# wing02/MyLdpcCppApi

Measured on AMD Instinct MI355X. Metric: decoded Mbit/s (info bits), DVB-S2 N=64800 rate-1/2, 50 iters, higher is better.
Workload: dtype f32; 1 GPU; DVB-S2-profile (64800,32400) rate-1/2 (seeded IRA table with the standard's structure, E=226799), batch 4096 frames per GPU, 50 iterations, sum-product fp32 (probability domain), all-zero codeword + AWGN sigma=0.95 (no frame converges), early termination on, inputs resident in HBM; global_batch=4096, frames_per_gpu=4096, algo=sp, frames_per_launch=4096, parallelism=frames sharded over 1 GPU(s), all-gather of decoded bytes, frames_converged=0

## Files before the change

### include/ldpc_hip.h

```cpp
#ifndef LDPC_HIP_H_
#define LDPC_HIP_H_

#include <stddef.h>
#include <stdint.h>

#ifdef __cplusplus
extern "C" {
#endif

#define LDPC_HIP_ABI_VERSION 3

enum ldpc_status {
    LDPC_OK = 0,
    LDPC_ERR_ARG = 1,
    LDPC_ERR_HIP = 2,
    LDPC_ERR_NOMEM = 3,
    LDPC_ERR_UNSUPPORTED = 4,
    LDPC_ERR_STATE = 5
};

enum ldpc_algo {
    LDPC_ALGO_SP = 0,
    LDPC_ALGO_MS = 1,
    LDPC_ALGO_LAYERED = 2,
    LDPC_ALGO_MS_FUSED = 3,
    LDPC_ALGO_LAYERED_HOST = 4
};

enum ldpc_msg_dtype { LDPC_MSG_F32 = 0, LDPC_MSG_F16 = 1 };

enum ldpc_host_input { LDPC_HOST_INPUT_AUTO = 0, LDPC_HOST_INPUT_STAGED = 1, LDPC_HOST_INPUT_LOCK_PAGES = 2 };

enum ldpc_pack_mode {
    LDPC_PACK_BYTES = 0,
    LDPC_PACK_BITS = 1
};

typedef struct ldpc_graph ldpc_graph;
typedef struct ldpc_decoder ldpc_decoder;

typedef struct ldpc_decoder_config {
    uint32_t struct_size;
    int32_t K;
    int32_t max_batch;
    int32_t algo;
    int32_t msg_dtype;
    int32_t max_iter;
    float llr_scale;
    int32_t early_term;
    int32_t device;
    int32_t layer_rows;
    int32_t pack_mode;
    int32_t frames_per_lane;
    int32_t poll_interval;
    int32_t tune_flags;
    int32_t tune_rows_per_wave;
    int32_t tune_cols_per_wave;
    int32_t tune_link_rows;
    int32_t tune_compact;
    int32_t tune_ldsp_grid;
    int32_t tune_ldsp_shape;
    int32_t tune_place;
    int32_t host_input;
    int32_t host_copy_threads;
    int32_t tune_q_order;
    float ms_scale;
    float ms_offset;
} ldpc_decoder_config;

enum ldpc_tune_field {
    LDPC_TUNE_FUSED = 0,
    LDPC_TUNE_LDSP = 2,
    LDPC_TUNE_LDSP_EXT = 4,
    LDPC_TUNE_LDSP_PACK = 6,
    LDPC_TUNE_LINK_NARROW = 8,
    LDPC_TUNE_CHECK_WIDE = 10,
    LDPC_TUNE_SYN_XCD = 12,
    LDPC_TUNE_FUSED_PACK = 14,
    LDPC_TUNE_FUSED_LOOP = 16,
    LDPC_TUNE_DEVICE_TAIL = 18,
    LDPC_TUNE_MERGE = 20,
    LDPC_TUNE_LINK_DEEP = 22,
    LDPC_TUNE_LINK_HALF = 24,
    LDPC_TUNE_LINK_GUIDED = 26,
    LDPC_TUNE_TILES_FIRST = 28
};
#define LDPC_TUNE_ON(field) (1 << (field))
#define LDPC_TUNE_OFF(field) (2 << (field))

typedef struct ldpc_decode_stats {
    int32_t iterations_launched;
    int32_t batch_time;
    int64_t frames;
    int64_t frames_converged;
    float ms_total;
    float ms_check;
    float ms_var;
    float ms_other;
    int32_t launches_check;
    int32_t launches_var;
    int64_t frame_rounds;
} ldpc_decode_stats;

int ldpc_abi_version(void);
const char *ldpc_last_error(void);
int ldpc_device_count(int *count);

int ldpc_graph_create(const int32_t *rows, const int32_t *cols, int64_t E, int32_t M, int32_t N,
                      ldpc_graph **out);
int ldpc_graph_destroy(ldpc_graph *g);
int ldpc_graph_info(const ldpc_graph *g, int32_t *M, int32_t *N, int64_t *E, int32_t *max_row_deg,
                    int32_t *max_col_deg);

void ldpc_decoder_config_init(ldpc_decoder_config *cfg);
int ldpc_decoder_create(const ldpc_graph *g, const ldpc_decoder_config *cfg, ldpc_decoder **out);
int ldpc_decoder_create_multi(const ldpc_graph *g, const ldpc_decoder_config *cfg, const int32_t *devices,
                              int32_t n_devices, ldpc_decoder **out);
int ldpc_decoder_destroy(ldpc_decoder *d);
int ldpc_shard_range(int64_t frames, int32_t part, int32_t parts, int32_t unit, int64_t *lo, int64_t *hi);

int ldpc_decode(ldpc_decoder *d, const float *llr_host, int64_t frames, uint8_t *out_host,
                int64_t out_bytes, int32_t *iters);

int ldpc_decode_device(ldpc_decoder *d, const float *llr_dev, int64_t frames, uint8_t *out_dev,
                       int64_t out_bytes, int32_t *iters_dev, void *stream);

int64_t ldpc_out_bytes(int32_t K, int64_t frames, int32_t pack_mode);

int ldpc_decoder_set_timing(ldpc_decoder *d, int enable);
int ldpc_decoder_stats(ldpc_decoder *d, ldpc_decode_stats *stats);

typedef struct ldpc_kernel_time {
    int32_t phase;
    int32_t degree;
    int32_t launches;
    float ms_total;
    int64_t bytes_total;
    char name[64];
    int64_t bytes_moved;
} ldpc_kernel_time;
int ldpc_decoder_kernel_times(ldpc_decoder *d, ldpc_kernel_time *out, int32_t capacity,
                              int32_t *count);

int ldpc_decoder_link_form(ldpc_decoder *d, int32_t *form, int32_t *calibrated, float ms[3]);

int ldpc_decoder_placement(ldpc_decoder *d, int32_t *candidates, int32_t *kept, float ms[16]);
int ldpc_decoder_array_addresses(ldpc_decoder *d, uint64_t out[4]);

int ldpc_decoder_set_tap(ldpc_decoder *d, int32_t iter);
int ldpc_decoder_dump(ldpc_decoder *d, int32_t which, float *host_out, int64_t count);

int ldpc_awgn_device(float *llr_dev, int64_t frames, int32_t N, const uint8_t *bits_dev, float sd,
                     uint64_t seed, int64_t first_frame, int32_t device, void *stream);
int ldpc_count_errors_device(const uint8_t *out_dev, const uint8_t *ref_dev, int64_t frames,
                             int64_t bytes_per_frame, int64_t errors[3], int32_t device, void *stream);

typedef struct ldpc_encoder ldpc_encoder;
enum ldpc_code_format {
    LDPC_CODE_PACKED = 0,
    LDPC_CODE_BITS = 1
};
enum ldpc_parity_kind { LDPC_PARITY_DUAL_DIAGONAL = 1, LDPC_PARITY_STAIRCASE = 2 };
int ldpc_parity_structure(const ldpc_graph *g, int32_t K, int32_t block_rows, int32_t out[8]);
int ldpc_encoder_create(const ldpc_graph *g, int32_t K, int32_t block_rows, int32_t max_frames, int32_t device,
                        ldpc_encoder **out);
int ldpc_encoder_destroy(ldpc_encoder *e);
int ldpc_encode_device(ldpc_encoder *e, const uint8_t *src_dev, int64_t src_bytes, int64_t frames, uint8_t *code_dev,
                       int64_t code_bytes, int32_t format, void *stream);
int ldpc_encode(ldpc_encoder *e, const uint8_t *src_host, int64_t src_bytes, uint8_t *code_host, int64_t code_bytes);
int64_t ldpc_code_bytes(int32_t N, int64_t frames, int32_t format);

int ldpc_hbm_probe_device(int32_t device, int64_t bytes, int32_t reps, double *copy_gbs, double *by_policy);
int ldpc_hbm_sustained_device(int32_t device, int64_t bytes, int32_t milliseconds, double *copy_gbs);

int ldpc_host_block_plan(uint64_t base, int64_t frames, int32_t N, int32_t max_batch, int64_t group, uint64_t out[6]);
int ldpc_host_locked_ranges(int64_t *live, int64_t *stale);

#ifdef __cplusplus
}
#endif
#endif
```

### myldpccppapi_amd/_lib.py

```python
import ctypes
import os
import sys

_HERE = os.path.dirname(os.path.abspath(__file__))
LIB_PATH = os.environ.get("LDPC_HIP_LIB") or os.path.join(_HERE, "libldpc_hip.so")
_lib = None


class LdpcError(RuntimeError):
    def __init__(self, code, message):
        super().__init__("ldpc_hip error %d: %s" % (code, message))
        self.code = code


class DecoderConfig(ctypes.Structure):
    _fields_ = [("struct_size", ctypes.c_uint32), ("K", ctypes.c_int32),
                ("max_batch", ctypes.c_int32), ("algo", ctypes.c_int32),
                ("msg_dtype", ctypes.c_int32), ("max_iter", ctypes.c_int32),
                ("llr_scale", ctypes.c_float), ("early_term", ctypes.c_int32),
                ("device", ctypes.c_int32), ("layer_rows", ctypes.c_int32),
                ("pack_mode", ctypes.c_int32), ("frames_per_lane", ctypes.c_int32),
                ("poll_interval", ctypes.c_int32),
                ("tune_flags", ctypes.c_int32), ("tune_rows_per_wave", ctypes.c_int32),
                ("tune_cols_per_wave", ctypes.c_int32), ("tune_link_rows", ctypes.c_int32),
                ("tune_compact", ctypes.c_int32), ("tune_ldsp_grid", ctypes.c_int32),
                ("tune_ldsp_shape", ctypes.c_int32), ("tune_place", ctypes.c_int32),
                ("host_input", ctypes.c_int32),
                ("host_copy_threads", ctypes.c_int32), ("tune_q_order", ctypes.c_int32),
                ("ms_scale", ctypes.c_float), ("ms_offset", ctypes.c_float)]


class DecodeStats(ctypes.Structure):
    _fields_ = [("iterations_launched", ctypes.c_int32), ("batch_time", ctypes.c_int32),
                ("frames", ctypes.c_int64), ("frames_converged", ctypes.c_int64),
                ("ms_total", ctypes.c_float), ("ms_check", ctypes.c_float),
                ("ms_var", ctypes.c_float), ("ms_other", ctypes.c_float),
                ("launches_check", ctypes.c_int32), ("launches_var", ctypes.c_int32),
                ("frame_rounds", ctypes.c_int64)]


class KernelTime(ctypes.Structure):
    _fields_ = [("phase", ctypes.c_int32), ("degree", ctypes.c_int32), ("launches", ctypes.c_int32),
                ("ms_total", ctypes.c_float), ("bytes_total", ctypes.c_int64), ("name", ctypes.c_char * 64),
                ("bytes_moved", ctypes.c_int64)]


EXPORTS = (
    "ldpc_abi_version", "ldpc_last_error", "ldpc_device_count", "ldpc_graph_create",
    "ldpc_graph_destroy", "ldpc_graph_info", "ldpc_decoder_config_init", "ldpc_decoder_create",
    "ldpc_decoder_create_multi", "ldpc_shard_range", "ldpc_decoder_destroy", "ldpc_decode", "ldpc_decode_device", "ldpc_out_bytes",
    "ldpc_decoder_set_timing", "ldpc_decoder_stats", "ldpc_decoder_kernel_times", "ldpc_decoder_set_tap",
    "ldpc_decoder_dump", "ldpc_awgn_device", "ldpc_count_errors_device", "ldpc_hbm_probe_device", "ldpc_hbm_sustained_device",
    "ldpc_host_block_plan", "ldpc_host_locked_ranges", "ldpc_decoder_link_form", "ldpc_decoder_placement", "ldpc_decoder_array_addresses",
    "ldpc_parity_structure", "ldpc_encoder_create", "ldpc_encoder_destroy", "ldpc_encode_device", "ldpc_encode", "ldpc_code_bytes",
)


def load():
    global _lib
    if _lib is not None:
        return _lib
    if not os.path.exists(LIB_PATH):
        raise OSError("%s not built: run `python -c 'import __graft_entry__ as g; g.build()'` "
                      "or `make -C myldpccppapi_amd/csrc`" % LIB_PATH)
    if "torch" not in sys.modules:
        try:
            import torch
        except Exception:
            pass
    L = ctypes.CDLL(LIB_PATH, mode=ctypes.RTLD_GLOBAL)
    i32p = ctypes.POINTER(ctypes.c_int32)
    i64p = ctypes.POINTER(ctypes.c_int64)
    vp = ctypes.c_void_p
    L.ldpc_abi_version.restype = ctypes.c_int
    L.ldpc_last_error.restype = ctypes.c_char_p
    L.ldpc_device_count.argtypes = [ctypes.POINTER(ctypes.c_int)]
    L.ldpc_graph_create.argtypes = [i32p, i32p, ctypes.c_int64, ctypes.c_int32, ctypes.c_int32,
                                    ctypes.POINTER(vp)]
    L.ldpc_graph_destroy.argtypes = [vp]
    L.ldpc_graph_info.argtypes = [vp, i32p, i32p, i64p, i32p, i32p]
    L.ldpc_decoder_config_init.argtypes = [ctypes.POINTER(DecoderConfig)]
    L.ldpc_decoder_config_init.restype = None
    L.ldpc_decoder_create.argtypes = [vp, ctypes.POINTER(DecoderConfig), ctypes.POINTER(vp)]
    L.ldpc_decoder_create_multi.argtypes = [vp, ctypes.POINTER(DecoderConfig), i32p, ctypes.c_int32,
                                            ctypes.POINTER(vp)]
    L.ldpc_shard_range.argtypes = [ctypes.c_int64, ctypes.c_int32, ctypes.c_int32, ctypes.c_int32, i64p, i64p]
    L.ldpc_decoder_destroy.argtypes = [vp]
    L.ldpc_decode.argtypes = [vp, vp, ctypes.c_int64, vp, ctypes.c_int64, vp]
    L.ldpc_decode_device.argtypes = [vp, vp, ctypes.c_int64, vp, ctypes.c_int64, vp, vp]
    L.ldpc_out_bytes.argtypes = [ctypes.c_int32, ctypes.c_int64, ctypes.c_int32]
    L.ldpc_out_bytes.restype = ctypes.c_int64
    L.ldpc_decoder_set_timing.argtypes = [vp, ctypes.c_int]
    L.ldpc_decoder_stats.argtypes = [vp, ctypes.POINTER(DecodeStats)]
    L.ldpc_decoder_kernel_times.argtypes = [vp, ctypes.POINTER(KernelTime), ctypes.c_int32, i32p]
    L.ldpc_decoder_set_tap.argtypes = [vp, ctypes.c_int32]
    L.ldpc_decoder_dump.argtypes = [vp, ctypes.c_int32, vp, ctypes.c_int64]
    L.ldpc_awgn_device.argtypes = [vp, ctypes.c_int64, ctypes.c_int32, vp, ctypes.c_float, ctypes.c_uint64,
                                   ctypes.c_int64, ctypes.c_int32, vp]
    L.ldpc_count_errors_device.argtypes = [vp, vp, ctypes.c_int64, ctypes.c_int64, i64p, ctypes.c_int32, vp]
    L.ldpc_hbm_sustained_device.argtypes = [ctypes.c_int32, ctypes.c_int64, ctypes.c_int32, ctypes.POINTER(ctypes.c_double)]
    L.ldpc_hbm_probe_device.argtypes = [ctypes.c_int32, ctypes.c_int64, ctypes.c_int32,
                                        ctypes.POINTER(ctypes.c_double), ctypes.POINTER(ctypes.c_double)]
    L.ldpc_host_block_plan.argtypes = [ctypes.c_uint64, ctypes.c_int64, ctypes.c_int32, ctypes.c_int32, ctypes.c_int64,
                                       ctypes.POINTER(ctypes.c_uint64)]
    L.ldpc_host_locked_ranges.argtypes = [i64p, i64p]
    L.ldpc_decoder_array_addresses.argtypes = [vp, ctypes.POINTER(ctypes.c_uint64)]
    L.ldpc_decoder_placement.argtypes = [vp, i32p, i32p, ctypes.POINTER(ctypes.c_float)]
    L.ldpc_decoder_link_form.argtypes = [vp, i32p, i32p, ctypes.POINTER(ctypes.c_float)]
    L.ldpc_parity_structure.argtypes = [vp, ctypes.c_int32, ctypes.c_int32, i32p]
    L.ldpc_encoder_create.argtypes = [vp, ctypes.c_int32, ctypes.c_int32, ctypes.c_int32, ctypes.c_int32, ctypes.POINTER(vp)]
    L.ldpc_encoder_destroy.argtypes = [vp]
    L.ldpc_encode_device.argtypes = [vp, vp, ctypes.c_int64, ctypes.c_int64, vp, ctypes.c_int64, ctypes.c_int32, vp]
    L.ldpc_encode.argtypes = [vp, vp, ctypes.c_int64, vp, ctypes.c_int64]
    L.ldpc_code_bytes.argtypes = [ctypes.c_int32, ctypes.c_int64, ctypes.c_int32]
    L.ldpc_code_bytes.restype = ctypes.c_int64
    _lib = L
    return L


def check(rc):
    if rc != 0:
        raise LdpcError(rc, load().ldpc_last_error().decode("utf-8", "replace"))
```

### myldpccppapi_amd/capi.py

```python
import ctypes

import numpy as np

from . import _lib
from ._lib import DecoderConfig, DecodeStats, LdpcError

ALGO_SP, ALGO_MS, ALGO_LAYERED, ALGO_MS_FUSED, ALGO_LAYERED_HOST = 0, 1, 2, 3, 4
MSG_F32, MSG_F16 = 0, 1
PACK_BYTES, PACK_BITS = 0, 1
CODE_PACKED, CODE_BITS = 0, 1
CODE_FORMATS = {"packed": CODE_PACKED, "bits": CODE_BITS}
PARITY_KINDS = {1: "dual_diagonal", 2: "staircase"}
HOST_INPUT = {"auto": 0, "staged": 1, "lock_pages": 2}
ALGOS = {"sp": ALGO_SP, "ms": ALGO_MS, "layered": ALGO_LAYERED, "ms_fused": ALGO_MS_FUSED,
         "layered_host": ALGO_LAYERED_HOST}

TUNE_FIELDS = {"fused": 0, "ldsp": 2, "ldsp_ext": 4, "ldsp_pack": 6, "link_narrow": 8, "check_wide": 10,
               "syn_xcd": 12, "fused_pack": 14, "fused_loop": 16, "device_tail": 18, "merge": 20, "link_deep": 22, "link_half": 24,
               "link_guided": 26, "tiles_first": 28}
TUNE_INTS = ("rows_per_wave", "cols_per_wave", "link_rows", "compact", "ldsp_grid", "ldsp_per_cu", "ldsp_waves", "place", "q_order")


def apply_tune(cfg, tune):
    flags, shape = 0, 0
    for k, v in (tune or {}).items():
        if k in TUNE_FIELDS:
            if v is not None:
                flags |= (1 if v else 2) << TUNE_FIELDS[k]
        elif k == "ldsp_per_cu":
            shape |= int(v) & 255
        elif k == "ldsp_waves":
            shape |= (int(v) & 255) << 8
        elif k in TUNE_INTS:
            setattr(cfg, "tune_" + k, int(v))
        else:
            raise KeyError("unknown tuning field %r" % k)
    cfg.tune_flags, cfg.tune_ldsp_shape = flags, shape


def hbm_probe(device=0, nbytes=1 << 30, reps=5, by_policy=False):
    g = ctypes.c_double(0.0)
    two = (ctypes.c_double * 2)(0.0, 0.0)
    _lib.check(_lib.load().ldpc_hbm_probe_device(int(device), int(nbytes), int(reps), ctypes.byref(g), two))
    return (g.value, two[0], two[1]) if by_policy else g.value


def hbm_sustained(device=0, nbytes=1 << 30, milliseconds=300):
    g = ctypes.c_double(0.0)
    _lib.check(_lib.load().ldpc_hbm_sustained_device(int(device), int(nbytes), int(milliseconds), ctypes.byref(g)))
    return g.value


def tune_from_env(env=None):
    import os
    env = os.environ if env is None else env
    t = {}
    for name, key in (("FUSED", "fused"), ("LDSP", "ldsp"), ("LDSP_EXT", "ldsp_ext"), ("LDSP_PACK", "ldsp_pack"),
                      ("LINK_NARROW", "link_narrow"), ("CHECK_WIDE", "check_wide"), ("SYN_XCD", "syn_xcd"),
                      ("FUSED_LOOP", "fused_loop"), ("DEVICE_TAIL", "device_tail"), ("MERGE", "merge"), ("LINK_DEEP", "link_deep"), ("LINK_HALF", "link_half"),
                      ("LINK_GUIDED", "link_guided"), ("TILES_FIRST", "tiles_first")):
        if "LDPC_TUNE_" + name in env:
            t[key] = int(env["LDPC_TUNE_" + name]) != 0
    if "LDPC_TUNE_NO_PACK" in env:
        t["fused_pack"] = False
    for name, key in (("RPW", "rows_per_wave"), ("CPW", "cols_per_wave"), ("LDSP_GRID", "ldsp_grid"),
                      ("LDSP_PER_CU", "ldsp_per_cu"), ("LDSP_WAVES", "ldsp_waves")):
        if "LDPC_TUNE_" + name in env:
            t[key] = int(env["LDPC_TUNE_" + name])
    for name, key in (("LINK_RPW", "link_rows"), ("COMPACT", "compact")):
        if "LDPC_TUNE_" + name in env:
            v = int(env["LDPC_TUNE_" + name])
            t[key] = v if v > 0 else -1
    return t


def shard_range(frames, part, parts, unit=1):
    lo, hi = ctypes.c_int64(), ctypes.c_int64()
    _lib.check(_lib.load().ldpc_shard_range(int(frames), int(part), int(parts), int(unit),
                                            ctypes.byref(lo), ctypes.byref(hi)))
    return lo.value, hi.value


def host_block_plan(base, frames, N, max_batch, group):
    out = (ctypes.c_uint64 * 6)()
    _lib.check(_lib.load().ldpc_host_block_plan(int(base), int(frames), int(N), int(max_batch), int(group), out))
    return tuple(int(x) for x in out)


def host_locked_ranges():
    a, b = ctypes.c_int64(-1), ctypes.c_int64(-1)
    _lib.check(_lib.load().ldpc_host_locked_ranges(ctypes.byref(a), ctypes.byref(b)))
    return a.value, b.value


def device_count():
    n = ctypes.c_int(0)
    rc = _lib.load().ldpc_device_count(ctypes.byref(n))
    return n.value if rc == 0 else 0


def out_bytes(K, frames, pack_mode=PACK_BYTES):
    return int(_lib.load().ldpc_out_bytes(K, frames, pack_mode))


def code_bytes(N, frames, fmt="packed"):
    return int(_lib.load().ldpc_code_bytes(int(N), int(frames), CODE_FORMATS.get(fmt, fmt)))


def parity_structure(graph, K, block_rows=0):
    out = (ctypes.c_int32 * 8)()
    _lib.check(_lib.load().ldpc_parity_structure(graph._h, int(K), int(block_rows), out))
    return dict(kind=PARITY_KINDS[out[0]], c=out[1], x=out[2], a=out[3], b=out[4], ext_rows=out[5], z=out[6])


class Graph:

    def __init__(self, rows, cols, M, N):
        L = _lib.load()
        self.rows = np.ascontiguousarray(rows, np.int32)
        self.cols = np.ascontiguousarray(cols, np.int32)
        if self.rows.shape != self.cols.shape or self.rows.ndim != 1:
            raise ValueError("rows and cols must be 1-D arrays of equal length")
        self.M, self.N, self.E = int(M), int(N), int(self.rows.size)
        self._h = ctypes.c_void_p()
        i32p = ctypes.POINTER(ctypes.c_int32)
        _lib.check(L.ldpc_graph_create(self.rows.ctypes.data_as(i32p), self.cols.ctypes.data_as(i32p),
                                       self.E, self.M, self.N, ctypes.byref(self._h)))

    def info(self):
        L = _lib.load()
        M, N, rd, cd = (ctypes.c_int32() for _ in range(4))
        E = ctypes.c_int64()
        _lib.check(L.ldpc_graph_info(self._h, ctypes.byref(M), ctypes.byref(N), ctypes.byref(E),
                                     ctypes.byref(rd), ctypes.byref(cd)))
        return dict(M=M.value, N=N.value, E=E.value, max_row_deg=rd.value, max_col_deg=cd.value)

    def close(self):
        h, self._h = getattr(self, "_h", None), None
        if h and _lib is not None and _lib._lib is not None:
            _lib._lib.ldpc_graph_destroy(h)

    def __del__(self):
        try:
            self.close()
        except Exception:
            pass


class Decoder:

    def __init__(self, graph, K, max_batch, algo="sp", max_iter=40, llr_scale=8.0, early_term=True,
                 device=0, layer_rows=0, pack_mode=PACK_BYTES, frames_per_lane=0, poll_interval=0,
                 msg_dtype=MSG_F32, tune=None, devices=None, host_input="auto", host_copy_threads=0,
                 ms_scale=0.0, ms_offset=0.0):
        L = _lib.load()
        cfg = DecoderConfig()
        L.ldpc_decoder_config_init(ctypes.byref(cfg))
        cfg.K, cfg.max_batch = int(K), int(max_batch)
        cfg.algo = ALGOS[algo] if isinstance(algo, str) else int(algo)
        cfg.msg_dtype = {"f32": MSG_F32, "f16": MSG_F16}.get(msg_dtype, msg_dtype)
        cfg.max_iter, cfg.llr_scale = int(max_iter), float(llr_scale)
        cfg.early_term, cfg.device, cfg.layer_rows = int(bool(early_term)), int(device), int(layer_rows)
        cfg.pack_mode, cfg.frames_per_lane, cfg.poll_interval = int(pack_mode), int(frames_per_lane), int(poll_interval)
        apply_tune(cfg, tune)
        cfg.host_input = HOST_INPUT[host_input] if isinstance(host_input, str) else int(host_input)
        cfg.host_copy_threads = int(host_copy_threads)
        cfg.ms_scale, cfg.ms_offset = float(ms_scale), float(ms_offset)
        self.cfg = cfg
        self.graph = graph
        self.K, self.N, self.E = int(K), graph.N, graph.E
        self._h = ctypes.c_void_p()
        if devices is None:
            _lib.check(L.ldpc_decoder_create(graph._h, ctypes.byref(cfg), ctypes.byref(self._h)))
        else:
            devs = (ctypes.c_int32 * len(devices))(*[int(x) for x in devices])
            _lib.check(L.ldpc_decoder_create_multi(graph._h, ctypes.byref(cfg), devs, len(devices),
                                                   ctypes.byref(self._h)))

    def decode(self, llr, want_iters=True):
        L = _lib.load()
        llr = np.ascontiguousarray(llr, np.float32).reshape(-1, self.N)
        frames = llr.shape[0]
        out = np.zeros(out_bytes(self.K, frames, self.cfg.pack_mode), np.uint8)
        iters = np.zeros(frames, np.int32)
        _lib.check(L.ldpc_decode(self._h, llr.ctypes.data, frames, out.ctypes.data, out.size,
                                 iters.ctypes.data if want_iters else None))
        return out, iters

    def decode_device(self, llr_ptr, frames, out_ptr, out_nbytes, iters_ptr=None, stream=None):
        _lib.check(_lib.load().ldpc_decode_device(self._h, llr_ptr, frames, out_ptr, out_nbytes,
                                                  iters_ptr, stream))

    def set_timing(self, enable=True):
        _lib.check(_lib.load().ldpc_decoder_set_timing(self._h, int(enable)))

    def stats(self):
        st = DecodeStats()
        _lib.check(_lib.load().ldpc_decoder_stats(self._h, ctypes.byref(st)))
        return {f: getattr(st, f) for f, _ in st._fields_}

    def kernel_times(self):
        arr = (_lib.KernelTime * 64)()
        n = ctypes.c_int32(0)
        _lib.check(_lib.load().ldpc_decoder_kernel_times(self._h, arr, 64, ctypes.byref(n)))
        return [dict(name=arr[i].name.decode(), phase=arr[i].phase, degree=arr[i].degree,
                     launches=arr[i].launches, ms_total=arr[i].ms_total, bytes_total=arr[i].bytes_total,
                     bytes_moved=arr[i].bytes_moved)
                for i in range(n.value)]

    def link_form(self):
        form, cal = ctypes.c_int32(-1), ctypes.c_int32(0)
        ms = (ctypes.c_float * 3)()
        _lib.check(_lib.load().ldpc_decoder_link_form(self._h, ctypes.byref(form), ctypes.byref(cal), ms))
        if form.value < 0:
            return None
        return {"form": ("wide", "narrow", "half")[form.value], "chosen_by_measurement": bool(cal.value),
                "ms_per_launch": {"wide": round(ms[0], 4), "narrow": round(ms[1], 4), "half": round(ms[2], 4)}}

    def placement(self):
        n, kept = ctypes.c_int32(0), ctypes.c_int32(0)
        ms = (ctypes.c_float * 16)()
        _lib.check(_lib.load().ldpc_decoder_placement(self._h, ctypes.byref(n), ctypes.byref(kept), ms))
        if n.value == 0:
            return None
        return {"candidates_ms": [round(ms[i], 4) for i in range(n.value)], "kept": kept.value}

    def array_addresses(self):
        a = (ctypes.c_uint64 * 4)()
        _lib.check(_lib.load().ldpc_decoder_array_addresses(self._h, a))
        return {"Q": int(a[0]), "R": int(a[1]), "chan": int(a[2]), "hard": int(a[3])}

    def set_tap(self, it):
        _lib.check(_lib.load().ldpc_decoder_set_tap(self._h, int(it)))

    def dump(self, which, frames):
        per = self.N if which in (2, 3) else self.E
        a = np.empty((frames, per), np.float32)
        _lib.check(_lib.load().ldpc_decoder_dump(self._h, which, a.ctypes.data, a.size))
        return a

    def close(self):
        h, self._h = getattr(self, "_h", None), None
        if h and _lib is not None and _lib._lib is not None:
            _lib.check(_lib._lib.ldpc_decoder_destroy(h))

    def __del__(self):
        try:
            self.close()
        except Exception:
            pass


class Encoder:

    def __init__(self, graph, K, block_rows=0, max_frames=4096, device=0):
        L = _lib.load()
        self.graph, self.K, self.N = graph, int(K), graph.N
        self.block_rows, self.max_frames, self.device = int(block_rows), int(max_frames), int(device)
        self._h = ctypes.c_void_p()
        _lib.check(L.ldpc_encoder_create(graph._h, self.K, self.block_rows, self.max_frames, self.device,
                                         ctypes.byref(self._h)))

    def structure(self):
        return parity_structure(self.graph, self.K, self.block_rows)

    def encode(self, src_bytes):
        src = np.ascontiguousarray(np.frombuffer(bytes(src_bytes), np.uint8) if isinstance(src_bytes, (bytes, bytearray))
                                   else src_bytes, np.uint8).reshape(-1)
        frames = 1
        while frames * self.K // 8 < src.size:
            frames += 1
        out = np.zeros(code_bytes(self.N, frames, "packed"), np.uint8)
        _lib.check(_lib.load().ldpc_encode(self._h, src.ctypes.data, src.size, out.ctypes.data, out.size))
        return out

    def encode_device(self, src_ptr, src_nbytes, frames, code_ptr, code_nbytes, fmt="bits", stream=None):
        _lib.check(_lib.load().ldpc_encode_device(self._h, src_ptr, int(src_nbytes), int(frames), code_ptr,
                                                  int(code_nbytes), CODE_FORMATS.get(fmt, fmt), stream))

    def close(self):
        h, self._h = getattr(self, "_h", None), None
        if h and _lib is not None and _lib._lib is not None:
            _lib.check(_lib._lib.ldpc_encoder_destroy(h))

    def __del__(self):
        try:
            self.close()
        except Exception:
            pass
```

### myldpccppapi_amd/csrc/flood_kernels.hpp

```cpp
#pragma once

#include <hip/hip_runtime.h>
#include <stdint.h>

#include "ldpc_expf.h"

namespace ldpc {

constexpr int kAlgoSP = 0;
constexpr int kAlgoMS = 1;
constexpr int kAlgoMSC = 2;
constexpr int kCompactCapacity = 512;
constexpr int kLastCapacity = 64;
constexpr int kBlock = 256;
constexpr int kWavesPerBlock = 4;
constexpr int kMaxUnrolledDegree = 16;
constexpr int kMaxUnrolledCheckDegreeMS = 32;

#ifndef LDPC_NT_LOAD
#define LDPC_NT_LOAD 1
#endif
#ifndef LDPC_NT_STORE
#define LDPC_NT_STORE 1
#endif
// ... 58 lines not shown
    const vh4 t = ld_stream(reinterpret_cast<const vh4 *>(p));
    d[0] = (float)t.x; d[1] = (float)t.y; d[2] = (float)t.z; d[3] = (float)t.w;
}
template <int V> __device__ __forceinline__ void vstore(hf *p, const float (&s)[V]);
template <> __device__ __forceinline__ void vstore<1>(hf *p, const float (&s)[1]) { st_stream(p, (hf)s[0]); }
template <> __device__ __forceinline__ void vstore<2>(hf *p, const float (&s)[2])
{
    vh2 t; t.x = (hf)s[0]; t.y = (hf)s[1];
    st_stream(reinterpret_cast<vh2 *>(p), t);
}
template <> __device__ __forceinline__ void vstore<4>(hf *p, const float (&s)[4])
{
    vh4 t; t.x = (hf)s[0]; t.y = (hf)s[1]; t.z = (hf)s[2]; t.w = (hf)s[3];
    st_stream(reinterpret_cast<vh4 *>(p), t);
}

__device__ __forceinline__ int wave_id_in_block()
{
    return __builtin_amdgcn_readfirstlane((int)(threadIdx.x >> 6));
}

template <int V> __device__ __forceinline__ bool tile_finished(const uint64_t *done, int tile)
{
    bool all = true;
#pragma unroll
    for (int v = 0; v < V; ++v) all = all && (done[(size_t)tile * V + v] == ~0ull);
    return all;
}

struct TailRef {
    const int32_t *state;
    int32_t base_tile;
    int32_t n_tiles;
};

template <int V> __device__ __forceinline__ int tile_select(const TailRef &t, const uint64_t *done, int row)
{
    int tile = row;
    if (t.state && __builtin_amdgcn_readfirstlane(t.state[0])) {
        if (row >= t.n_tiles) return -1;
        tile = t.base_tile + row;
    }
    return tile_finished<V>(done, tile) ? -1 : tile;
}


struct CheckArgs {
    const void *__restrict__ Q;
    void *__restrict__ R;
    const int32_t *__restrict__ cls_e0;
    const uint64_t *__restrict__ done;
    int64_t E;
    int32_t n_rows;
    int32_t rows_per_wave;
    int32_t degree;
    float ms_scale = 1.0f;
    TailRef tail;
    int32_t tiles_first = 0;
    float ms_offset = 0.0f;
    const void *__restrict__ first_chan = nullptr;
    const int32_t *__restrict__ edge_col = nullptr;
    int32_t N = 0;
    const int32_t *__restrict__ qpos = nullptr;
};

template <int D> __device__ __forceinline__ void row_slots(const int32_t *__restrict__ qpos, int e0, int lane, int (&slot)[D])
{
    static_assert(D <= 64, "one lane per edge");
    const int mine = qpos[e0 + (lane < D ? lane : D - 1)];
#pragma unroll
    for (int k = 0; k < D; ++k) slot[k] = __builtin_amdgcn_readlane(mine, k);
}
__device__ __forceinline__ int edge_slot(const int32_t *__restrict__ qpos, int e)
{
    return __builtin_amdgcn_readfirstlane(qpos[e]);
}

struct GridPos { int row, block; };
__device__ __forceinline__ GridPos grid_pos(int tiles_first)
{
    return tiles_first ? GridPos{(int)blockIdx.x, (int)blockIdx.y} : GridPos{(int)blockIdx.y, (int)blockIdx.x};
}

template <int D, int V>
__device__ __forceinline__ void check_sp(const float (&x)[D][V], float (&out)[D][V])
{
#pragma unroll
    for (int v = 0; v < V; ++v) {
        if (D == 1) { out[0][v] = 1.0f; continue; }
        {
            float p = x[1][v];
#pragma unroll
            for (int j = 2; j < D; ++j) p *= x[j][v];
            out[0][v] = p;
        }
        float pre = x[0][v];
#pragma unroll
        for (int k = 1; k < D; ++k) {
            float p = pre;
#pragma unroll
            for (int j = k + 1; j < D; ++j) p *= x[j][v];
            out[k][v] = p;
            pre *= x[k][v];
        }
    }
}

struct MsCorr {
    float scale, offset;
};
template <typename T> __device__ __forceinline__ float ms_corr(float m, const MsCorr &c)
{
    const float r = fmaxf(m - c.offset, 0.0f) * c.scale;
    return sizeof(T) == 2 ? (float)(hf)r : r;
}

template <int D, int V, bool CORR = false, typename T = float>
__device__ __forceinline__ void check_ms(const float (&x)[D][V], float (&out)[D][V], MsCorr c = MsCorr{1.0f, 0.0f})
{
#pragma unroll
    for (int v = 0; v < V; ++v) {
        float m1 = 1000.0f, m2 = 1000.0f;
        int idx = -1;
        unsigned par = 0;
#pragma unroll
        for (int j = 0; j < D; ++j) {
            const float a = __builtin_fabsf(x[j][v]);
            par ^= (x[j][v] < 0.0f) ? 1u : 0u;
            if (a < m1) { m2 = m1; m1 = a; idx = j; }
            else if (a < m2) { m2 = a; }
        }
        if (CORR) { m1 = ms_corr<T>(m1, c); m2 = ms_corr<T>(m2, c); }
#pragma unroll
        for (int k = 0; k < D; ++k) {
            const float b = (k == idx) ? m2 : m1;
            const unsigned s = par ^ ((x[k][v] < 0.0f) ? 1u : 0u);
            out[k][v] = s ? -b : b;
        }
    }
}

__device__ __forceinline__ MsCorr ms_corr_of(const CheckArgs &a) { return MsCorr{a.ms_scale, a.ms_offset}; }

template <int ALGO, int D, int V, int W, typename T>
__global__ __launch_bounds__(kBlock) void check_kernel(const CheckArgs a)
{
    constexpr size_t F = 64 * V;
    constexpr int SUB = V / W;
    const int lane = threadIdx.x & 63;
    const GridPos gp = grid_pos(a.tiles_first);
    const int tile = tile_select<V>(a.tail, a.done, gp.row);
    if (tile < 0) return;
    const int wave = gp.block * kWavesPerBlock + wave_id_in_block();
    const int sub = wave % SUB;
    const int r_begin = (wave / SUB) * a.rows_per_wave;
    const int r_end = min(r_begin + a.rows_per_wave, a.n_rows);
    const unsigned lane_off = (unsigned)sub * 64 * W + (unsigned)lane * W;
    const T *Qu = static_cast<const T *>(a.Q) + (size_t)tile * (size_t)a.E * F;
    T *Rt = static_cast<T *>(a.R) + (size_t)tile * (size_t)a.E * F + lane_off;

    const T *Ct = (ALGO != kAlgoSP && a.first_chan)
                      ? static_cast<const T *>(a.first_chan) + (size_t)tile * (size_t)a.N * F + lane_off : nullptr;
    for (int r = r_begin; r < r_end; ++r) {
        const int e0 = a.cls_e0[r];
        float x[D][W], out[D][W];
        if (ALGO != kAlgoSP && Ct) {
#pragma unroll
            for (int k = 0; k < D; ++k) vload<W>(x[k], Ct + (size_t)a.edge_col[e0 + k] * F);
        } else {
            int sl[D];
            row_slots<D>(a.qpos, e0, lane, sl);
#pragma unroll
            for (int k = 0; k < D; ++k) vload<W>(x[k], Qu + (size_t)sl[k] * F + lane_off);
        }
        if (ALGO == kAlgoSP) check_sp<D, W>(x, out); else if (ALGO == kAlgoMS) check_ms<D, W>(x, out); else check_ms<D, W, true, T>(x, out, ms_corr_of(a));
#pragma unroll
        for (int k = 0; k < D; ++k) vstore<W>(Rt + (size_t)(e0 + k) * F, out[k]);
    }
}

template <int ALGO, int V, typename T>
__device__ __forceinline__ void check_row_generic(const T *Qu, unsigned lane_off, T *Rt, int e0, int D,
                                                  const int32_t *__restrict__ qpos, const MsCorr &c)
{
    constexpr size_t F = 64 * V;
    if (ALGO != kAlgoSP) {
        float m1[V], m2[V];
        int idx[V];
        unsigned par[V];
#pragma unroll
        for (int v = 0; v < V; ++v) { m1[v] = 1000.0f; m2[v] = 1000.0f; idx[v] = -1; par[v] = 0; }
        for (int j = 0; j < D; ++j) {
            float xj[V];
            vload<V>(xj, Qu + (size_t)edge_slot(qpos, e0 + j) * F + lane_off);
#pragma unroll
            for (int v = 0; v < V; ++v) {
                const float m = __builtin_fabsf(xj[v]);
                par[v] ^= (xj[v] < 0.0f) ? 1u : 0u;
                if (m < m1[v]) { m2[v] = m1[v]; m1[v] = m; idx[v] = j; }
                else if (m < m2[v]) { m2[v] = m; }
            }
        }
        if (ALGO == kAlgoMSC) {
#pragma unroll
            for (int v = 0; v < V; ++v) { m1[v] = ms_corr<T>(m1[v], c); m2[v] = ms_corr<T>(m2[v], c); }
        }
        for (int k = 0; k < D; ++k) {
            float xk[V], o[V];
            vload<V>(xk, Qu + (size_t)edge_slot(qpos, e0 + k) * F + lane_off);
#pragma unroll
            for (int v = 0; v < V; ++v) {
                const float b = (k == idx[v]) ? m2[v] : m1[v];
                const unsigned sg = par[v] ^ ((xk[v] < 0.0f) ? 1u : 0u);
                o[v] = sg ? -b : b;
            }
            vstore<V>(Rt + (size_t)(e0 + k) * F, o);
        }
        return;
    }
    for (int k = 0; k < D; ++k) {
        float o[V];
        float p[V];
#pragma unroll
        for (int v = 0; v < V; ++v) p[v] = 1.0f;
        for (int j = 0; j < D; ++j) {
            if (j == k) continue;
            float xj[V];
            vload<V>(xj, Qu + (size_t)edge_slot(qpos, e0 + j) * F + lane_off);
#pragma unroll
            for (int v = 0; v < V; ++v) p[v] *= xj[v];
        }
#pragma unroll
        for (int v = 0; v < V; ++v) o[v] = p[v];
        vstore<V>(Rt + (size_t)(e0 + k) * F, o);
    }
}

template <int ALGO, int V, typename T>
__global__ __launch_bounds__(kBlock) void check_kernel_generic(const CheckArgs a)
{
    constexpr size_t F = 64 * V;
    const int lane = threadIdx.x & 63;
    const GridPos gp = grid_pos(a.tiles_first);
    const int tile = tile_select<V>(a.tail, a.done, gp.row);
    if (tile < 0) return;
    const int wave = gp.block * kWavesPerBlock + wave_id_in_block();
    const int r_begin = wave * a.rows_per_wave;
    const int r_end = min(r_begin + a.rows_per_wave, a.n_rows);
    const T *Qu = static_cast<const T *>(a.Q) + (size_t)tile * (size_t)a.E * F;
    T *Rt = static_cast<T *>(a.R) + (size_t)tile * (size_t)a.E * F + (size_t)lane * V;
    for (int r = r_begin; r < r_end; ++r) check_row_generic<ALGO, V, T>(Qu, (unsigned)lane * V, Rt, a.cls_e0[r], a.degree, a.qpos, ms_corr_of(a));
}

struct GroupClass {
    int32_t block_begin;
    int32_t degree;
    int32_t count;
    int32_t pad;
    const int32_t *ids;
    const int32_t *edges;
    int64_t q_base;
};

template <int ALGO, int D, int V, int W, typename T>
__device__ __forceinline__ void check_rows(const T *Qu, unsigned lane_off, T *Rt, const int32_t *__restrict__ e0s, int r_begin, int r_end,
                                           const T *Ct, const int32_t *__restrict__ edge_col,
                                           const int32_t *__restrict__ qpos, const MsCorr &c)
{
    const int lane = threadIdx.x & 63;
    constexpr size_t F = 64 * V;
    for (int r = r_begin; r < r_end; ++r) {
        const int e0 = e0s[r];
        float x[D][W], out[D][W];
        if (ALGO != kAlgoSP && Ct) {
#pragma unroll
            for (int k = 0; k < D; ++k) vload<W>(x[k], Ct + (size_t)edge_col[e0 + k] * F);
        } else {
            int sl[D];
            row_slots<D>(qpos, e0, lane, sl);
#pragma unroll
            for (int k = 0; k < D; ++k) vload<W>(x[k], Qu + (size_t)sl[k] * F + lane_off);
        }
        if (ALGO == kAlgoSP) check_sp<D, W>(x, out); else if (ALGO == kAlgoMS) check_ms<D, W>(x, out); else check_ms<D, W, true, T>(x, out, c);
#pragma unroll
        for (int k = 0; k < D; ++k) vstore<W>(Rt + (size_t)(e0 + k) * F, out[k]);
    }
}

template <int ALGO, int V, typename T, int D, int DLO, int W = 1> struct CheckDispatch {
    static __device__ __forceinline__ void run(int deg, const T *Qu, unsigned lane_off, T *Rt, const int32_t *e0s, int rb, int re,
                                               const T *Ct, const int32_t *edge_col, const int32_t *qpos, const MsCorr &c)
    {
        if (deg == D) check_rows<ALGO, D, V, W, T>(Qu, lane_off, Rt, e0s, rb, re, Ct, edge_col, qpos, c);
        else CheckDispatch<ALGO, V, T, D - 1, DLO, W>::run(deg, Qu, lane_off, Rt, e0s, rb, re, Ct, edge_col, qpos, c);
    }
};
template <int ALGO, int V, typename T, int DLO, int W> struct CheckDispatch<ALGO, V, T, DLO, DLO, W> {
    static __device__ __forceinline__ void run(int, const T *Qu, unsigned lane_off, T *Rt, const int32_t *e0s, int rb, int re,
                                               const T *Ct, const int32_t *edge_col, const int32_t *qpos, const MsCorr &c)
    {
        check_rows<ALGO, DLO, V, W, T>(Qu, lane_off, Rt, e0s, rb, re, Ct, edge_col, qpos, c);
    }
};

template <int ALGO, int V, typename T, int DLO, int DHI, int W = 1>
__global__ __launch_bounds__(kBlock) void check_group_kernel(const CheckArgs a, const GroupClass *__restrict__ cls, int n_classes)
{
    constexpr size_t F = 64 * V;
    constexpr int SUB = V / W;
    const int lane = threadIdx.x & 63;
    const GridPos gp = grid_pos(a.tiles_first);
    const int tile = tile_select<V>(a.tail, a.done, gp.row);
    if (tile < 0) return;
    int c = 0;
    while (c + 1 < n_classes && gp.block >= cls[c + 1].block_begin) ++c;
    const int wave = (gp.block - cls[c].block_begin) * kWavesPerBlock + wave_id_in_block();
    const int sub = wave % SUB;
    const int r_begin = (wave / SUB) * a.rows_per_wave;
    const int r_end = min(r_begin + a.rows_per_wave, cls[c].count);
    const unsigned lane_off = (unsigned)sub * 64 * W + (unsigned)lane * W;
    const T *Qu = static_cast<const T *>(a.Q) + (size_t)tile * (size_t)a.E * F;
    T *Rt = static_cast<T *>(a.R) + (size_t)tile * (size_t)a.E * F + lane_off;
    const T *Ct = (ALGO != kAlgoSP && a.first_chan)
                      ? static_cast<const T *>(a.first_chan) + (size_t)tile * (size_t)a.N * F + lane_off : nullptr;
    CheckDispatch<ALGO, V, T, DHI, DLO, W>::run(cls[c].degree, Qu, lane_off, Rt, cls[c].ids, r_begin, r_end, Ct, a.edge_col, a.qpos, ms_corr_of(a));
}

struct SyndromeArgs {
    const int32_t *__restrict__ row_ptr;
    const int32_t *__restrict__ edge_col;
    const uint64_t *__restrict__ hard;
    uint64_t *__restrict__ fail;
    const uint64_t *__restrict__ done;
    int32_t M, N;
    int32_t tiles;
    int32_t row_blocks;
    TailRef tail;
};

template <int V> __global__ __launch_bounds__(kBlock) void syndrome_kernel(const SyndromeArgs a)
{
    int tile, rb;
    if (a.tiles > 0) {
        const int xcd = blockIdx.x & 7, j = blockIdx.x >> 3;
        tile = xcd + 8 * (j / a.row_blocks);
        rb = j % a.row_blocks;
        if (tile >= a.tiles) return;
    } else {
        tile = blockIdx.y;
        rb = blockIdx.x;
    }
    tile = tile_select<V>(a.tail, a.done, tile);
    if (tile < 0) return;
    const int m = rb * kBlock + threadIdx.x;
    const uint64_t *hard_t = a.hard + (size_t)tile * (size_t)a.N * V;
    uint64_t s[V];
#pragma unroll
    for (int v = 0; v < V; ++v) s[v] = 0;
    if (m < a.M) {
        for (int p = a.row_ptr[m]; p < a.row_ptr[m + 1]; ++p) {
            const int c = a.edge_col[p];
#pragma unroll
            for (int v = 0; v < V; ++v) s[v] ^= hard_t[(size_t)c * V + v];
        }
    }
    __shared__ uint64_t part[kWavesPerBlock][V];
#pragma unroll
    for (int v = 0; v < V; ++v) {
        uint64_t x = s[v];
#pragma unroll
        for (int off = 32; off >= 1; off >>= 1) {
            const uint32_t lo = __shfl_xor((uint32_t)x, off);
            const uint32_t hi = __shfl_xor((uint32_t)(x >> 32), off);
            x |= ((uint64_t)hi << 32) | lo;
        }
        if ((threadIdx.x & 63) == 0) part[threadIdx.x >> 6][v] = x;
    }
    __syncthreads();
    if (threadIdx.x < V) {
        uint64_t x = 0;
#pragma unroll
        for (int w = 0; w < kWavesPerBlock; ++w) x |= part[w][threadIdx.x];
        unsigned long long *dst = reinterpret_cast<unsigned long long *>(&a.fail[(size_t)tile * V + threadIdx.x]);
        const uint64_t seen = __hip_atomic_load(dst, __ATOMIC_RELAXED, __HIP_MEMORY_SCOPE_AGENT);
        if (x & ~seen) atomicOr(dst, (unsigned long long)x);
    }
}


struct VarArgs {
    const void *__restrict__ R;
    void *__restrict__ Q;
    const void *__restrict__ chan;
    uint64_t *hard;
    const uint64_t *__restrict__ done;
    const int32_t *__restrict__ cls_col;
    const int32_t *__restrict__ cls_edge;
    int64_t E;
    int32_t N;
    int32_t n_cols;
    int32_t cols_per_wave;
    int32_t write_q;
    int32_t degree;
    TailRef tail;
    int32_t tiles_first = 0;
    int64_t q_base = -1;
};

template <int D, int V>
__device__ __forceinline__ void var_sp(const float (&t)[V], const float (&d)[D][V],
                                       float (&outq)[D][V], float (&full0)[V], float (&full1)[V])
{
#pragma unroll
    for (int v = 0; v < V; ++v) {
        const float den = 1.0f + t[v];
        float pre0 = t[v] / den;
        float pre1 = 1.0f / den;
        float r0[D], r1[D];
#pragma unroll
        for (int k = 0; k < D; ++k) {
            r0[k] = (1.0f + d[k][v]) * 0.5f;
            r1[k] = (1.0f - d[k][v]) * 0.5f;
        }
#pragma unroll
        for (int k = 0; k < D; ++k) {
            float t0 = pre0, t1 = pre1;
#pragma unroll
            for (int j = k + 1; j < D; ++j) { t0 *= r0[j]; t1 *= r1[j]; }
            const float s = t0 + t1;
            const float q0 = t0 / s;
            const float q1 = t1 / s;
            outq[k][v] = q0 - q1;
            pre0 *= r0[k];
            pre1 *= r1[k];
        }
        full0[v] = pre0;
        full1[v] = pre1;
    }
}

struct LinkArgs {
    const int32_t *__restrict__ link_col;
    const int32_t *__restrict__ link_pos;
    const void *__restrict__ chan;
    void *Qw;
    uint64_t *hard;
    int32_t N;
    int32_t write_q;
    int32_t store_all;
    const int32_t *__restrict__ extra_e0;
    const int32_t *__restrict__ extra_deg;
    int32_t n_extra;
    int32_t link_blocks;
    int32_t n_big, small_rows;
};

__host__ __device__ inline void link_chunk_rows(int c, int rows_per_wave, int n_big, int small_rows, int n_rows,
                                               int *rb, int *re)
{
    int b, e;
    if (c < n_big) { b = c * rows_per_wave; e = b + rows_per_wave; }
    else { b = n_big * rows_per_wave + (c - n_big) * small_rows; e = b + small_rows; }
    *rb = b < n_rows ? b : n_rows;
    *re = e < n_rows ? e : n_rows;
}
__host__ __device__ inline int link_chunk_count(int rows_per_wave, int n_big, int small_rows, int n_rows)
{
    const int rest = n_rows - n_big * rows_per_wave;
    return n_big + (rest > 0 ? (rest + small_rows - 1) / small_rows : 0);
}

template <int ALGO, int V, typename T>
__device__ __forceinline__ void link_extra_rows(const CheckArgs &a, const LinkArgs &g, int tile, int block)
{
    constexpr size_t F = 64 * V;
    const int lane = threadIdx.x & 63;
    const int w = (block - g.link_blocks) * kWavesPerBlock + wave_id_in_block();
    if (w >= g.n_extra) return;
    const T *Qu = static_cast<const T *>(a.Q) + (size_t)tile * (size_t)a.E * F;
    T *Rt = static_cast<T *>(a.R) + (size_t)tile * (size_t)a.E * F + (size_t)lane * V;
    check_row_generic<ALGO, V, T>(Qu, (unsigned)lane * V, Rt, g.extra_e0[w], g.extra_deg[w], a.qpos, ms_corr_of(a));
}

#ifdef LDPC_LINK_WIDE_WAVES
#define LDPC_LINK_WIDE_ATTR __attribute__((amdgpu_waves_per_eu(LDPC_LINK_WIDE_WAVES, LDPC_LINK_WIDE_WAVES)))
#else
#define LDPC_LINK_WIDE_ATTR
#endif
template <int ALGO, int D, int V, typename T>
__global__ __launch_bounds__(kBlock) LDPC_LINK_WIDE_ATTR void check_link_kernel(const CheckArgs a, const LinkArgs g)
{
    constexpr size_t F = 64 * V;
    const int lane = threadIdx.x & 63;
    const GridPos gp = grid_pos(a.tiles_first);
    const int tile = tile_select<V>(a.tail, a.done, gp.row);
    if (tile < 0) return;
    if (gp.block >= g.link_blocks) { link_extra_rows<ALGO, V, T>(a, g, tile, gp.block); return; }
    const int wave = gp.block * kWavesPerBlock + wave_id_in_block();
    int r_begin, r_end;
    link_chunk_rows(wave, a.rows_per_wave, g.n_big, g.small_rows, a.n_rows, &r_begin, &r_end);
    const size_t lane_off = (size_t)lane * V;
    const unsigned lane_q = (unsigned)lane * V;
    const T *Qt = static_cast<const T *>(a.Q) + (size_t)tile * (size_t)a.E * F;
    T *Qwt = static_cast<T *>(g.Qw) + (size_t)tile * (size_t)a.E * F;
    T *Rt = static_cast<T *>(a.R) + (size_t)tile * (size_t)a.E * F + lane_off;
    const T *chan_t = static_cast<const T *>(g.chan) + (size_t)tile * (size_t)g.N * F + lane_off;
    uint64_t *hard_t = g.hard + (size_t)tile * (size_t)g.N * V;
    uint64_t frozen[V];
#pragma unroll
    for (int v = 0; v < V; ++v) frozen[v] = a.done[(size_t)tile * V + v];

    int pend_col = -1, pend_edge = 0, pend_kb = 0;
    float pend_r[V];
#pragma unroll
    for (int v = 0; v < V; ++v) pend_r[v] = 0.0f;

    float x[D][V];
    int qc[D], qn[D];
#pragma unroll
    for (int k = 0; k < D; ++k) qc[k] = qn[k] = 0;
    if (r_begin < r_end) {
        row_slots<D>(a.qpos, a.cls_e0[r_begin], lane, qc);
#pragma unroll
        for (int k = 0; k < D; ++k) vload<V>(x[k], Qt + (size_t)qc[k] * F + lane_q);
    }
    for (int r = r_begin; r < r_end; ++r) {
        const int e0 = a.cls_e0[r];
        const int next_col = (r + 1 < r_end) ? g.link_col[r] : -1;
        const int pos = g.link_pos[r];
        const int ka = next_col >= 0 ? (pos & 255) : -1;
        const int kb = pend_col >= 0 ? pend_kb : -1;
        if (r + 1 < r_end) row_slots<D>(a.qpos, a.cls_e0[r + 1], lane, qn);
        float ch[V];
        uint64_t old_w[V];
        if (pend_col >= 0) {
            vload<V>(ch, chan_t + (size_t)pend_col * F);
#pragma unroll
            for (int v = 0; v < V; ++v) old_w[v] = hard_t[(size_t)pend_col * V + v];
        }
        float out[D][V];
        if (ALGO == kAlgoSP) check_sp<D, V>(x, out); else if (ALGO == kAlgoMS) check_ms<D, V>(x, out); else check_ms<D, V, true, T>(x, out, ms_corr_of(a));
        if (r + 1 < r_end) {
#pragma unroll
            for (int k = 0; k < D; ++k) vload<V>(x[k], Qt + (size_t)qn[k] * F + lane_q);
        }
#pragma unroll
        for (int k = 0; k < D; ++k)
            if ((k != ka && k != kb) || g.store_all) vstore<V>(Rt + (size_t)(e0 + k) * F, out[k]);

        if (pend_col >= 0) {
            float rr[2][V], q[2][V];
#pragma unroll
            for (int v = 0; v < V; ++v) {
                rr[0][v] = pend_r[v];
                float t = out[0][v];
#pragma unroll
                for (int k = 1; k < D; ++k) t = (k == kb) ? out[k][v] : t;
                rr[1][v] = t;
            }
            uint64_t new_w[V];
            if (ALGO == kAlgoSP) {
                float f0[V], f1[V];
                var_sp<2, V>(ch, rr, q, f0, f1);
#pragma unroll
                for (int v = 0; v < V; ++v) {
                    const bool oldb = (old_w[v] >> lane) & 1ull;
                    const bool b = (f0[v] > f1[v]) ? false : ((f0[v] < f1[v]) ? true : oldb);
                    new_w[v] = __ballot(b);
                }
            } else {
#pragma unroll
                for (int v = 0; v < V; ++v) {
                    float p = ch[v];
                    p += rr[0][v];
                    p += rr[1][v];
                    q[0][v] = p - rr[0][v];
                    q[1][v] = p - rr[1][v];
                    new_w[v] = __ballot(!(p > 0.0f));
                }
            }
            if (lane == 0) {
#pragma unroll
                for (int v = 0; v < V; ++v)
                    hard_t[(size_t)pend_col * V + v] = (old_w[v] & frozen[v]) | (new_w[v] & ~frozen[v]);
            }
            if (g.write_q) {
                int qw1 = qc[0];
#pragma unroll
                for (int k = 1; k < D; ++k) qw1 = (k == kb) ? qc[k] : qw1;
                vstore<V>(Qwt + (size_t)pend_edge * F + lane_q, q[0]);
                vstore<V>(Qwt + (size_t)qw1 * F + lane_q, q[1]);
            }
        }
        pend_col = next_col;
        if (next_col >= 0) {
            pend_edge = qc[0];
#pragma unroll
            for (int k = 1; k < D; ++k) pend_edge = (k == ka) ? qc[k] : pend_edge;
            pend_kb = (pos >> 8) & 255;
#pragma unroll
            for (int v = 0; v < V; ++v) {
                float t = out[0][v];
#pragma unroll
                for (int k = 1; k < D; ++k) t = (k == ka) ? out[k][v] : t;
                pend_r[v] = t;
            }
        }
#pragma unroll
        for (int k = 0; k < D; ++k) qc[k] = qn[k];
    }
}

template <int V> __device__ __forceinline__ uint64_t compress_stride(uint64_t x)
{
    if (V == 1) return x;
    if (V == 2) {
        x &= 0x5555555555555555ull;
        x = (x | (x >> 1)) & 0x3333333333333333ull;
        x = (x | (x >> 2)) & 0x0f0f0f0f0f0f0f0full;
        x = (x | (x >> 4)) & 0x00ff00ff00ff00ffull;
        x = (x | (x >> 8)) & 0x0000ffff0000ffffull;
        x = (x | (x >> 16)) & 0x00000000ffffffffull;
        return x;
    }
    x &= 0x1111111111111111ull;
    x = (x | (x >> 3)) & 0x0303030303030303ull;
    x = (x | (x >> 6)) & 0x000f000f000f000full;
// ... 466 lines not shown
#pragma unroll
            for (int v = 0; v < V; ++v) new_w[v] = __ballot(!(p[v] > 0.0f));
            if (a.write_q) {
                for (int j = 0; j < D; ++j) {
                    float rj[V], o[V];
                    vload<V>(rj, Rt + (size_t)e[j] * F);
#pragma unroll
                    for (int v = 0; v < V; ++v) o[v] = p[v] - rj[v];
                    vstore<V>(Qt + qs(j) * F, o);
                }
            }
        }
        if (lane == 0) {
#pragma unroll
            for (int v = 0; v < V; ++v)
                hard_t[(size_t)n * V + v] = (old_w[v] & frozen[v]) | (new_w[v] & ~frozen[v]);
        }
    }
}


struct InitArgs {
    const float *__restrict__ llr;
    void *__restrict__ chan;
    void *__restrict__ Q;
    uint64_t *__restrict__ hard;
    const int32_t *__restrict__ col_ptr;
    const int32_t *__restrict__ col_edge;
    int64_t E;
    int64_t frames;
    int32_t N;
    float llr_scale;
};

constexpr int kInitCols = 32;

template <int ALGO, int V, typename T>
__global__ __launch_bounds__(kBlock) void init_kernel(const InitArgs a)
{
    constexpr int F = 64 * V;
    constexpr int LD = F + 1;
    __shared__ float patch[kInitCols * LD];
    const int tile = blockIdx.y;
    const int n0 = blockIdx.x * kInitCols;
    if ((a.N & 3) == 0 && n0 + kInitCols <= a.N && (reinterpret_cast<uintptr_t>(a.llr) & 15) == 0) {
        const int c4 = (threadIdx.x & 7) * 4, f0 = threadIdx.x >> 3;
        float4 vals[F / 32];
#pragma unroll
        for (int i = 0; i < F / 32; ++i) {
            const int64_t frame = (int64_t)tile * F + f0 + 32 * i;
            vals[i] = float4{1.0f, 1.0f, 1.0f, 1.0f};
            if (frame < a.frames) vals[i] = *reinterpret_cast<const float4 *>(a.llr + (size_t)frame * a.N + n0 + c4);
        }
#pragma unroll
        for (int i = 0; i < F / 32; ++i) {
            const int f = f0 + 32 * i;
            patch[(c4 + 0) * LD + f] = vals[i].x;
            patch[(c4 + 1) * LD + f] = vals[i].y;
            patch[(c4 + 2) * LD + f] = vals[i].z;
            patch[(c4 + 3) * LD + f] = vals[i].w;
        }
    } else {
        const int c = threadIdx.x & (kInitCols - 1);
        const int n = n0 + c;
        for (int f = threadIdx.x / kInitCols; f < F; f += kBlock / kInitCols) {
            const int64_t frame = (int64_t)tile * F + f;
            float y = 1.0f;
            if (frame < a.frames && n < a.N) y = a.llr[(size_t)frame * a.N + n];
            patch[c * LD + f] = y;
        }
    }
    __syncthreads();
    const int lane = threadIdx.x & 63;
    for (int c = threadIdx.x >> 6; c < kInitCols; c += kWavesPerBlock) {
        const int n = n0 + c;
        if (n >= a.N) break;
        float ch[V], q[V];
#pragma unroll
        for (int v = 0; v < V; ++v) {
            const float y = patch[c * LD + lane * V + v];
            if (ALGO == kAlgoSP) {
                const float t = ldpc_expf(a.llr_scale * y);
                ch[v] = t;
                q[v] = t / (1.0f + t) - 1.0f / (1.0f + t);
            } else {
                ch[v] = y;
                q[v] = y;
            }
        }
        vstore<V>(static_cast<T *>(a.chan) + ((size_t)tile * a.N + n) * F + (size_t)lane * V, ch);
        if (a.Q) {
            const int p0 = a.col_ptr[n], deg = a.col_ptr[n + 1] - p0;
            T *Qt = static_cast<T *>(a.Q) + (size_t)tile * (size_t)a.E * F + (size_t)lane * V;
            for (int k0 = 0; k0 < deg; k0 += 64) {
                const int m = min(64, deg - k0);
                const int mine = a.col_edge[p0 + k0 + (lane < m ? lane : m - 1)];
                for (int k = 0; k < m; ++k)
                    vstore<V>(Qt + (size_t)__builtin_amdgcn_readlane(mine, k) * F, q);
            }
        }
        if (lane < V) a.hard[((size_t)tile * a.N + n) * V + lane] = 0;
    }
}

struct StateArgs {
    uint64_t *__restrict__ done;
    const uint64_t *__restrict__ fail;
    int32_t *__restrict__ iters;
    int32_t *__restrict__ active;
    int64_t frames;
    int32_t iter;
    int32_t max_iter;
    int32_t freeze;
    TailRef tail;
    int32_t *__restrict__ running;
    int32_t *__restrict__ tile_rounds;
};

template <int V> __global__ void state_kernel(const StateArgs a)
{
    constexpr int F = 64 * V;
    int tile = blockIdx.x;
    if (a.tail.state && a.iter > 0 && a.tail.state[0]) {
        if (tile >= a.tail.n_tiles) return;
        tile = a.tail.base_tile + tile;
    }
    const int lane = threadIdx.x;
    int n_active = 0;
    bool worked = false;
#pragma unroll
    for (int v = 0; v < V; ++v) {
        const int64_t frame = (int64_t)tile * F + (int64_t)lane * V + v;
        const bool valid = frame < a.frames;
        uint64_t d;
        if (a.iter == 0) {
            d = __ballot(!valid);
            a.iters[(size_t)tile * F + lane * V + v] = a.max_iter;
        } else {
            const uint64_t old = a.done[(size_t)tile * V + v];
            worked = worked || old != ~0ull;
            const uint64_t clean = ~a.fail[(size_t)tile * V + v];
            const uint64_t newly = clean & ~old;
            if ((newly >> lane) & 1ull) a.iters[(size_t)tile * F + lane * V + v] = a.iter;
            d = a.freeze ? (old | clean) : old;
        }
        if (lane == 0) a.done[(size_t)tile * V + v] = d;
        n_active += __popcll(~d);
    }
    if (lane == 0 && n_active && a.active) atomicAdd(a.active, n_active);
    if (lane == 0 && n_active && a.running) atomicAdd(&a.running[a.iter], n_active);
    if (lane == 0 && worked && a.tile_rounds) atomicAdd(a.tile_rounds, 1);
}

template <int V> __global__ __launch_bounds__(kBlock) void compact_list_kernel(const uint64_t *__restrict__ done, int64_t frames,
                                                                               int32_t *__restrict__ map, int32_t *__restrict__ count,
                                                                               int32_t capacity)
{
    constexpr int F = 64 * V;
    const int64_t f = (int64_t)blockIdx.x * kBlock + threadIdx.x;
    if (f >= frames) return;
    const int64_t tile = f / F;
    const int fi = (int)(f % F);
    if ((done[tile * V + fi % V] >> (fi / V)) & 1ull) return;
    const int slot = atomicAdd(count, 1);
    if (slot < capacity) map[slot] = (int32_t)f;
}

// ... 435 lines not shown
```

### myldpccppapi_amd/csrc/flood_tables.hpp

```cpp
#pragma once

#include "flood_kernels.hpp"

namespace ldpc {

using CheckFn = void (*)(const CheckArgs);
using VarFn = void (*)(const VarArgs);
using LinkFn = void (*)(const CheckArgs, const LinkArgs);
using CheckGroupFn = void (*)(const CheckArgs, const GroupClass *, int);
using VarGroupFn = void (*)(const VarArgs, const GroupClass *, int);
using InitFn = void (*)(const InitArgs);

constexpr int kVarBuckets = 3, kCheckBuckets = 4;
constexpr int kVarBucketLo[kVarBuckets] = {1, 5, 9}, kVarBucketHi[kVarBuckets] = {4, 8, 16};
constexpr int kCheckBucketLo[kCheckBuckets] = {1, 9, 17, 25}, kCheckBucketHi[kCheckBuckets] = {8, 16, 24, 32};

struct FloodFns {
    CheckFn check[kMaxUnrolledCheckDegreeMS + 1] = {};
    CheckFn check_wide[kMaxUnrolledCheckDegreeMS + 1] = {};
    LinkFn link[kMaxUnrolledDegree + 1] = {};
    LinkFn link_narrow[kMaxUnrolledDegree + 1] = {};
    LinkFn link_deep[kMaxUnrolledDegree + 1] = {};
    LinkFn link_half[kMaxUnrolledDegree + 1] = {};
    VarFn var[kMaxUnrolledDegree + 1] = {};
    CheckGroupFn check_group[kCheckBuckets] = {};
    int check_group_width = 1;
    VarGroupFn var_group[kVarBuckets] = {};
    InitFn init = nullptr;
    int max_check_unrolled = kMaxUnrolledDegree;
};

void fill_flood_sp(int V, FloodFns *f);
void fill_flood_ms(int V, FloodFns *f);
void fill_flood_ms16(int V, FloodFns *f);
void fill_flood_msc(int V, FloodFns *f);
void fill_flood_msc16(int V, FloodFns *f);

}
```

### myldpccppapi_amd/csrc/flood_tables_impl.hpp

```cpp
#pragma once

#include "flood_tables.hpp"

namespace ldpc {
namespace tables {

template <int ALGO, int V, typename T, int D> struct FloodTable {
    static void fill(CheckFn *c, CheckFn *cw, VarFn *v)
    {
        c[D] = check_kernel<ALGO, D, V, 1, T>;
        cw[D] = check_kernel<ALGO, D, V, V, T>;
        v[D] = var_kernel<ALGO, D, V, T>;
        FloodTable<ALGO, V, T, D - 1>::fill(c, cw, v);
    }
};
template <int ALGO, int V, typename T> struct FloodTable<ALGO, V, T, 0> {
    static void fill(CheckFn *c, CheckFn *cw, VarFn *v)
    {
        c[0] = cw[0] = check_kernel_generic<ALGO, V, T>;
        v[0] = var_kernel_generic<ALGO, V, T>;
    }
};

template <int ALGO, int V, typename T, int D> struct CheckTableMS {
    static void fill(CheckFn *c, CheckFn *cw)
    {
        c[D] = cw[D] = check_kernel<ALGO, D, V, 1, T>;
        CheckTableMS<ALGO, V, T, D - 1>::fill(c, cw);
    }
};
template <int ALGO, int V, typename T> struct CheckTableMS<ALGO, V, T, kMaxUnrolledDegree> {
    static void fill(CheckFn *, CheckFn *) {}
};

template <int ALGO, int V, typename T, int D> struct LinkHalf {
    static LinkFn get() { return nullptr; }
};
template <int ALGO, typename T, int D> struct LinkHalf<ALGO, 4, T, D> {
    static LinkFn get() { return check_link_narrow_kernel<ALGO, D, 4, T, 2>; }
};
template <int ALGO, int V, typename T, int D> struct LinkTable {
    static void fill(LinkFn *t, LinkFn *tn, LinkFn *td, LinkFn *th)
    {
        t[D] = check_link_kernel<ALGO, D, V, T>;
        tn[D] = check_link_narrow_kernel<ALGO, D, V, T>;
        td[D] = check_link_narrow2_kernel<ALGO, D, V, T>;
        th[D] = LinkHalf<ALGO, V, T, D>::get();
        LinkTable<ALGO, V, T, D - 1>::fill(t, tn, td, th);
    }
};
template <int ALGO, int V, typename T> struct LinkTable<ALGO, V, T, 1> {
    static void fill(LinkFn *, LinkFn *, LinkFn *, LinkFn *) {}
};

template <int ALGO, int V, typename T> void fill_v(FloodFns *f)
{
    constexpr int DM = kMaxUnrolledDegree;
    FloodTable<ALGO, V, T, DM>::fill(f->check, f->check_wide, f->var);
    LinkTable<ALGO, V, T, DM>::fill(f->link, f->link_narrow, f->link_deep, f->link_half);
    constexpr int GW = (sizeof(T) == 2 && V == 4) ? 2 : 1;
    f->check_group_width = GW;
    f->check_group[0] = check_group_kernel<ALGO, V, T, 1, 8, GW>;
    f->check_group[1] = check_group_kernel<ALGO, V, T, 9, 16, GW>;
    f->check_group[2] = f->check_group[3] = nullptr;
    f->var_group[0] = var_group_kernel<ALGO, V, T, 1, 4>;
    f->var_group[1] = var_group_kernel<ALGO, V, T, 5, 8>;
    f->var_group[2] = var_group_kernel<ALGO, V, T, 9, 16>;
    f->init = init_kernel<ALGO, V, T>;
    f->max_check_unrolled = DM;
    if (ALGO != kAlgoSP) {
        CheckTableMS<ALGO, V, T, kMaxUnrolledCheckDegreeMS>::fill(f->check, f->check_wide);
        f->check_group[2] = check_group_kernel<ALGO, V, T, 17, 24, GW>;
        f->check_group[3] = check_group_kernel<ALGO, V, T, 25, 32, GW>;
        f->max_check_unrolled = kMaxUnrolledCheckDegreeMS;
    }
}

template <int ALGO, typename T> void fill(int V, FloodFns *f)
{
    *f = FloodFns();
    if (V == 1) fill_v<ALGO, 1, T>(f);
    else if (V == 2) fill_v<ALGO, 2, T>(f);
    else fill_v<ALGO, 4, T>(f);
}

}
}
```

### myldpccppapi_amd/csrc/layered_kernels.hpp

```cpp
#pragma once

#include <hip/hip_runtime.h>
#include <stdint.h>

#include <map>
#include <vector>

#include "flood_kernels.hpp"

namespace ldpc {

struct LayerArgs {
    float *__restrict__ P;
    float *__restrict__ R;
    const int32_t *__restrict__ cls_e0;
    const int32_t *__restrict__ edge_col;
    uint64_t *hard;
    const uint64_t *__restrict__ done;
    int64_t E;
    int32_t N;
    int32_t n_rows;
    int32_t rows_per_wave;
    int32_t degree;
};
// ... 94 lines not shown
        for (int v = 0; v < V; ++v) {
            const uint64_t w = __ballot(y[v] < 0.0f);
            if (lane == 0) a.hard[((size_t)tile * a.N + n) * V + v] = a.zero_bits ? 0ull : w;
        }
    }
}


constexpr int kMaxUnrolledLayerDegree = 24;

struct LayerGroup {
    int layer = 0, degree = 0, count = 0;
    int32_t *e0 = nullptr;
};

struct LayeredPlan {
    int32_t M = 0, N = 0, layer_rows = 0;
    int64_t E = 0;
    int T = 0, V = 1;
    int host_arith = 0;
    int corr = 0;
    float ms_scale = 1.0f, ms_offset = 0.0f;
    float *P = nullptr, *R = nullptr;
    std::vector<LayerGroup> groups;
};

inline void layered_plan_destroy(LayeredPlan *pl)
{
    for (auto &g : pl->groups)
        if (g.e0) (void)hipFree(g.e0);
    pl->groups.clear();
    if (pl->P) (void)hipFree(pl->P);
    if (pl->R) (void)hipFree(pl->R);
    pl->P = pl->R = nullptr;
}

inline int layered_plan_create(LayeredPlan *pl, int32_t M, int32_t N, int64_t E,
                               const std::vector<int32_t> &row_ptr, const std::vector<int32_t> &cols,
                               int32_t layer_rows, int T, int V)
{
    if (layer_rows <= 0 || M % layer_rows) return -1;
    pl->M = M; pl->N = N; pl->E = E; pl->layer_rows = layer_rows; pl->T = T; pl->V = V;
    std::vector<int32_t> seen((size_t)N, -1);
    const int layers = M / layer_rows;
    for (int l = 0; l < layers; ++l) {
        std::map<int, std::vector<int32_t>> by_deg;
        for (int32_t m = l * layer_rows; m < (l + 1) * layer_rows; ++m) {
            for (int32_t p = row_ptr[m]; p < row_ptr[m + 1]; ++p) {
                if (seen[cols[p]] == l) return -1;
                seen[cols[p]] = l;
            }
            const int deg = row_ptr[m + 1] - row_ptr[m];
            if (deg > 0) by_deg[deg].push_back(row_ptr[m]);
        }
        for (auto &kv : by_deg) {
            LayerGroup g;
            g.layer = l; g.degree = kv.first; g.count = (int)kv.second.size();
            if (hipMalloc((void **)&g.e0, kv.second.size() * sizeof(int32_t)) != hipSuccess) return -2;
            pl->groups.push_back(g);
            if (hipMemcpy(g.e0, kv.second.data(), kv.second.size() * sizeof(int32_t),
                          hipMemcpyHostToDevice) != hipSuccess) return -2;
        }
    }
    const size_t TF = (size_t)T * 64 * V;
    if (hipMalloc((void **)&pl->P, TF * N * sizeof(float)) != hipSuccess) return -2;
    if (hipMalloc((void **)&pl->R, TF * (size_t)E * sizeof(float)) != hipSuccess) return -2;
    return 0;
}

struct LayeredRun {
    hipError_t (*span_begin)(void *ctx, hipStream_t s, int kind, int degree, int64_t bytes) = nullptr;
    hipError_t (*span_end)(void *ctx, hipStream_t s) = nullptr;
    void *span_ctx = nullptr;
    const float *llr_dev;
    int64_t frames;
    uint8_t *out_dev;
    int64_t out_bytes;
    int32_t *iters_dev;
    int32_t K, max_iter, tap_iter, early_term, pack_mode;
    uint64_t *hard, *failw, *done;
    int32_t *iters;
    const int32_t *row_ptr, *edge_col;
    int32_t *summary;
};

#ifdef LDPC_ENGINE_LAYERED
using LayerFn = void (*)(const LayerArgs);
template <int V, int D, bool HOST = false> struct LayerTable {
    static void fill(LayerFn *t) { t[D] = layer_kernel<D, V, HOST>; LayerTable<V, D - 1, HOST>::fill(t); }
};
template <int V, bool HOST> struct LayerTable<V, 0, HOST> {
    static void fill(LayerFn *t) { t[0] = HOST ? nullptr : layer_kernel_generic<V>; }
};
using LayerCorrFn = void (*)(const LayerArgs, const MsCorr);
template <int V, int D> struct LayerCorrTable {
    static void fill(LayerCorrFn *t) { t[D] = layer_corr_kernel<D, V>; LayerCorrTable<V, D - 1>::fill(t); }
};
template <int V> struct LayerCorrTable<V, 0> {
    static void fill(LayerCorrFn *t) { t[0] = layer_corr_kernel_generic<V>; }
};


template <int V> __global__ void layered_summary_kernel(const int32_t *iters, const uint64_t *done,
                                                        int64_t frames, int32_t *summary)
{
    constexpr int F = 64 * V;
    const int64_t f = (int64_t)blockIdx.x * blockDim.x + threadIdx.x;
    if (f >= frames) return;
    const int64_t tile = f / F;
    const int fi = (int)(f % F);
    atomicMax(&summary[0], iters[f]);
    if ((done[tile * V + fi % V] >> (fi / V)) & 1ull) atomicAdd(&summary[1], 1);
}

template <int V>
inline hipError_t layered_run_v(LayeredPlan *pl, const LayeredRun &r, hipStream_t s, int32_t *launched)
{
    constexpr int F = 64 * V;
    const int tiles = (int)((r.frames + F - 1) / F);
    const size_t slot = (size_t)pl->T * V;
    LayerFn table[kMaxUnrolledLayerDegree + 1];
    LayerCorrFn corr_table[kMaxUnrolledLayerDegree + 1];
    if (pl->host_arith) LayerTable<V, kMaxUnrolledLayerDegree, true>::fill(table);
    else LayerTable<V, kMaxUnrolledLayerDegree>::fill(table);
    LayerCorrTable<V, kMaxUnrolledLayerDegree>::fill(corr_table);
    const MsCorr corr{pl->ms_scale, pl->ms_offset};
    const int rounds = r.tap_iter ? (r.tap_iter < r.max_iter ? r.tap_iter : r.max_iter) : r.max_iter;
    hipError_t e;
    if ((e = hipMemsetAsync(r.failw, 0, (size_t)(r.max_iter + 2) * slot * sizeof(uint64_t), s))) return e;
    if ((e = hipMemsetAsync(r.summary, 0, 2 * sizeof(int32_t), s))) return e;
    if ((e = hipMemsetAsync(pl->R, 0, (size_t)tiles * F * (size_t)pl->E * sizeof(float), s))) return e;
    {
        LayeredInitArgs ia{r.llr_dev, pl->P, r.hard, r.frames, pl->N, pl->host_arith};
        dim3 grid((pl->N + kInitCols - 1) / kInitCols, tiles);
        layered_init_kernel<V><<<grid, kBlock, 0, s>>>(ia);
        StateArgs st{r.done, nullptr, r.iters, nullptr, r.frames, 0, r.max_iter, 1};
        state_kernel<V><<<tiles, 64, 0, s>>>(st);
    }
    int it = 0;
    for (it = 1; it <= rounds; ++it) {
        for (auto &g : pl->groups) {
            LayerArgs a{pl->P, pl->R, g.e0, r.edge_col, r.hard, r.done, pl->E, pl->N, g.count,
                        4, g.degree};
            const int waves = (g.count + a.rows_per_wave - 1) / a.rows_per_wave;
            dim3 grid((waves + kWavesPerBlock - 1) / kWavesPerBlock, tiles);
            const int k = g.degree <= kMaxUnrolledLayerDegree ? g.degree : 0;
            if (!table[k]) return hipErrorInvalidValue;
            if (r.span_begin && (e = r.span_begin(r.span_ctx, s, 2, g.degree,
                                                  (int64_t)16 * g.degree * g.count * r.frames))) return e;
            if (pl->corr) corr_table[k]<<<grid, kBlock, 0, s>>>(a, corr);
            else table[k]<<<grid, kBlock, 0, s>>>(a);
            if (r.span_end && (e = r.span_end(r.span_ctx, s))) return e;
        }
        if (pl->host_arith) {
            dim3 hgrid((pl->N + kWavesPerBlock - 1) / kWavesPerBlock, tiles);
            layered_hard_kernel<V><<<hgrid, kBlock, 0, s>>>(pl->P, r.hard, r.done, pl->N);
        }
        if (!r.early_term && it != rounds) continue;
        uint64_t *fw = r.failw + (size_t)it * slot;
        SyndromeArgs sa{r.row_ptr, r.edge_col, r.hard, fw, r.done, pl->M, pl->N, 0, 0};
        dim3 sgrid((pl->M + kBlock - 1) / kBlock, tiles);
        syndrome_kernel<V><<<sgrid, kBlock, 0, s>>>(sa);
        StateArgs st{r.done, fw, r.iters, nullptr, r.frames, it, r.max_iter, 1};
        state_kernel<V><<<tiles, 64, 0, s>>>(st);
    }
    *launched = rounds;
    PackArgs pa{r.hard, r.out_dev, r.iters, r.iters_dev, r.frames, r.out_bytes, pl->N, r.K, r.pack_mode};
    if (r.out_dev) {
        if (r.pack_mode == 0) {
            pack_kernel<V><<<pack_grid<V>(r.K, tiles), kBlock, 0, s>>>(pa);
        } else {
            const int64_t n = r.out_bytes > r.frames ? r.out_bytes : r.frames;
            pack_kernel<V><<<(unsigned)((n + kBlock - 1) / kBlock), kBlock, 0, s>>>(pa);
        }
    }
    layered_summary_kernel<V><<<(unsigned)((r.frames + 255) / 256), 256, 0, s>>>(r.iters, r.done, r.frames,
                                                                                 r.summary);
    return hipGetLastError();
}

inline hipError_t layered_run(LayeredPlan *pl, const LayeredRun &r, hipStream_t s, int32_t *launched)
{
    if (pl->V == 1) return layered_run_v<1>(pl, r, s, launched);
    if (pl->V == 2) return layered_run_v<2>(pl, r, s, launched);
    return layered_run_v<4>(pl, r, s, launched);
}

#endif

inline hipError_t layered_dump(LayeredPlan *pl, int which, float *host_out, int64_t count, int64_t frames,
                               const uint64_t *hard_dev, const int32_t *)
{
    const int V = pl->V, F = 64 * V;
    const int tiles = (int)((frames + F - 1) / F);
    if (which == 0 || which == 2) {
        const int64_t per = which == 0 ? pl->E : pl->N;
        if (count != frames * per) return hipErrorInvalidValue;
        const float *src = which == 0 ? pl->R : pl->P;
        std::vector<float> tile((size_t)per * F);
        for (int t = 0; t < tiles; ++t) {
            hipError_t e = hipMemcpy(tile.data(), src + (size_t)t * per * F, tile.size() * sizeof(float),
                                     hipMemcpyDeviceToHost);
            if (e != hipSuccess) return e;
            for (int fi = 0; fi < F; ++fi) {
                const int64_t f = (int64_t)t * F + fi;
                if (f >= frames) break;
                for (int64_t i = 0; i < per; ++i) host_out[f * per + i] = tile[(size_t)i * F + fi];
            }
        }
        return hipSuccess;
    }
    if (which == 3) {
        if (count != frames * pl->N) return hipErrorInvalidValue;
        std::vector<uint64_t> w((size_t)tiles * pl->N * V);
        hipError_t e = hipMemcpy(w.data(), hard_dev, w.size() * sizeof(uint64_t), hipMemcpyDeviceToHost);
        if (e != hipSuccess) return e;
        for (int64_t f = 0; f < frames; ++f) {
            const int64_t t = f / F;
            const int fi = (int)(f % F);
            for (int32_t n = 0; n < pl->N; ++n)
                host_out[f * pl->N + n] = (float)((w[((size_t)t * pl->N + n) * V + fi % V] >> (fi / V)) & 1ull);
        }
        return hipSuccess;
    }
    return hipErrorInvalidValue;
}

}
```

### myldpccppapi_amd/csrc/ldpc_hip.hip

```cpp
#include <hip/hip_runtime.h>

#include <algorithm>
#include <chrono>
#include <cstdarg>
#include <cstdio>
#include <cstdlib>
#include <cstring>
#include <map>
#include <memory>
#include <new>
#include <string>
#include <thread>
#include <vector>

#include "../../include/ldpc_hip.h"
#include "flood_kernels.hpp"
#include "flood_tables.hpp"
#include "layered_kernels.hpp"
#include "fused_kernels.hpp"
#include "ldsp_kernels.hpp"
#include "engines.hpp"
#include "channel_kernels.hpp"
#include "tune.hpp"
#include "host_stage.hpp"
// ... 80 lines not shown

using ldpc::CheckFn;
using ldpc::VarFn;
using ldpc::LinkFn;
using ldpc::CheckGroupFn;
using ldpc::VarGroupFn;
using ldpc::InitFn;
using ldpc::kVarBuckets;
using ldpc::kCheckBuckets;
using ldpc::kVarBucketLo;
using ldpc::kVarBucketHi;
using ldpc::kCheckBucketLo;
using ldpc::kCheckBucketHi;

struct RowClass {
    int degree = 0;
    int count = 0;
    DevBuf<int32_t> e0;
    std::vector<int32_t> h_e0;
    DevBuf<int32_t> link_col, link_pos;
    int linked = 0;
    int n_big = 0, small_rows = 1;
};
struct ColClass {
    int degree = 0;
    int count = 0;
    DevBuf<int32_t> col, edge;
    int64_t q_base = -1;
};

struct ClassGroup {
    int bucket = 0, lo = 0, hi = 0;
    int blocks = 0;
    int blocks_fat = 0;
    std::vector<int> members;
    DevBuf<ldpc::GroupClass> table, table_fat;
};

constexpr int kIdleFat = LDPC_IDLE_FAT;

struct TimedSpan {
    hipEvent_t a, b;
    int kind;
    int degree;
    int64_t bytes;
    int64_t moved;
    int lo;
};

}

struct ldpc_decoder {
    ldpc_decoder_config cfg{};
    int32_t M = 0, N = 0;
    int64_t E = 0;
    int V = 1, F = 64, T = 0;
    std::vector<int32_t> h_col_ptr, h_col_edge, h_rows, h_cols;

    DevBuf<int32_t> row_ptr, edge_col, col_ptr, col_edge;
    DevBuf<int32_t> qpos, col_qedge;
    std::vector<int32_t> h_qpos;
    DevBuf<uint8_t> chan, Q, R;
    int msg_size = 4;
    InitFn init_fn = nullptr;
    DevBuf<uint64_t> hard, failw, done;
    DevBuf<int32_t> iters, active;
    std::vector<RowClass> row_classes;
    std::vector<ColClass> col_classes;
    std::vector<ClassGroup> check_groups, var_groups;
    std::vector<int> check_solo, var_solo;
    CheckGroupFn check_group_fn[kCheckBuckets] = {};
    int check_group_width = 1;
    VarGroupFn var_group_fn[kVarBuckets] = {};
    DevBuf<int32_t> extra_e0, extra_deg;
    int n_extra = 0;
    int64_t extra_edges = 0;
    CheckFn check_fn[ldpc::kMaxUnrolledCheckDegreeMS + 1] = {};
    CheckFn check_fn_wide[ldpc::kMaxUnrolledCheckDegreeMS + 1] = {};
    int max_check_unrolled = ldpc::kMaxUnrolledDegree;
    LinkFn link_fn[ldpc::kMaxUnrolledDegree + 1] = {};
    LinkFn link_narrow_fn[ldpc::kMaxUnrolledDegree + 1] = {};
    LinkFn link_deep_fn[ldpc::kMaxUnrolledDegree + 1] = {};
    LinkFn link_half_fn[ldpc::kMaxUnrolledDegree + 1] = {};
    int tune_link_deep = 0;
    ldpc::Tune tune;
    int tune_link_narrow = 1;
    bool link_calibrated = false;
    float link_cal_ms[3] = {0, 0, 0};
    int place_candidates = 0, place_kept = 0;
    float place_ms[16] = {};
    int link_rpw = 16;
    int tune_link_guided = 0;
    int tune_tiles_first = 0;
    int cus = 256;
    VarFn var_fn[ldpc::kMaxUnrolledDegree + 1] = {};

    ldpc::LayeredPlan layered;
    ldpc::FusedPlan fused;
    bool use_fused = false;
    ldpc::LdspPlan ldsp;
    bool use_ldsp = false;
    bool ms_corr = false;
    float ms_scale = 1.0f, ms_offset = 0.0f;

    hipStream_t stream = nullptr, copy_stream = nullptr;
    struct HostSlot {
        DevBuf<float> llr;
        DevBuf<uint8_t> out;
        DevBuf<int32_t> iters;
        uint8_t *h_out = nullptr;
        int32_t *h_iters = nullptr;
        uint8_t *h_head = nullptr;
        hipEvent_t h2d_done = nullptr, all_done = nullptr;
        bool busy = false;
        int64_t off = 0, n = 0, dst = 0, copy_bytes = 0;
        int32_t *h_sum = nullptr;
        int g_iterations = 0, g_tiles = 0, g_children = 0, g_child_f[3] = {0, 0, 0};
    } slot[3];
    struct CallCounts { bool valid = false; int32_t iterations = 0, batch_time = 0; int64_t frames = 0, converged = 0, frame_rounds = 0; } call;
    bool suppress_poll = false;
    int32_t *h_active = nullptr;
    struct RingChunk { uint8_t *h = nullptr; hipEvent_t ev = nullptr; bool used = false; };
    std::vector<RingChunk> ring;
    size_t ring_next = 0;
    std::unique_ptr<ldpc::Worker> stager;
    std::vector<std::unique_ptr<ldpc::Worker>> copy_helpers;
    std::vector<ldpc::Job> copy_jobs;
    ldpc::Job stage_job[3];
    bool stage_pending[3] = {false, false, false};
    std::vector<void *> locked_blocks, stuck_blocks;
    ldpc_decoder *child = nullptr;
    DevBuf<int32_t> cmap;
    DevBuf<int32_t> cinv;
    DevBuf<unsigned long long> cmoved;
    int child_capacity = ldpc::kCompactCapacity;
    int compact_threshold = ldpc::kCompactCapacity;
    bool is_child = false;
    bool tail_enabled = false;
    int TO = 0, TA = 0;
    DevBuf<int32_t> tail_state, tail_map, running;
    int32_t *h_summary = nullptr;
    hipEvent_t ev_summary = nullptr;
    bool summary_pending = false;
    int idle_after = 0;

    bool timing = false;
    int timing_every = 0;
    int64_t timing_calls = 0;
    std::vector<TimedSpan> spans;
    size_t spans_used = 0;
    hipEvent_t ev_begin = nullptr, ev_end = nullptr;
    hipStream_t last_stream = nullptr;
    bool have_last = false;
    int32_t tap_iter = 0;
    int tune_rpw = 0, tune_cpw = 0;
    int tune_syn_xcd = 1;
    int tune_check_wide = 0;
    int32_t last_iterations = 0;
    int64_t last_frames = 0;
    DevBuf<int32_t> summary;
    ldpc_decoder *handed_to = nullptr;
    bool first_round_from_chan = false;
    int32_t last_tiles = 0;

    std::vector<ldpc_decoder *> shards;
    std::vector<std::unique_ptr<ldpc::Worker>> shard_workers;

    ~ldpc_decoder()
    {
        for (auto &w : shard_workers) w->stop();
        if (stager) stager->stop();
        for (auto &w : copy_helpers) w->stop();
        for (ldpc_decoder *sh : shards) (void)ldpc_decoder_destroy(sh);
        for (auto &s : spans) { (void)hipEventDestroy(s.a); (void)hipEventDestroy(s.b); }
        if (ev_begin) (void)hipEventDestroy(ev_begin);
        if (ev_end) (void)hipEventDestroy(ev_end);
        if (h_active) (void)hipHostFree(h_active);
        for (auto &rc : ring) {
            if (rc.h) (void)hipHostFree(rc.h);
            if (rc.ev) (void)hipEventDestroy(rc.ev);
        }
        if (h_summary) (void)hipHostFree(h_summary);
        if (ev_summary) (void)hipEventDestroy(ev_summary);
        for (auto &sl : slot) {
            if (sl.h_out) (void)hipHostFree(sl.h_out);
            if (sl.h_iters) (void)hipHostFree(sl.h_iters);
            if (sl.h_head) (void)hipHostFree(sl.h_head);
            if (sl.h_sum) (void)hipHostFree(sl.h_sum);
            if (sl.h2d_done) (void)hipEventDestroy(sl.h2d_done);
            if (sl.all_done) (void)hipEventDestroy(sl.all_done);
        }
        if (copy_stream) (void)hipStreamDestroy(copy_stream);
        if (stream) (void)hipStreamDestroy(stream);
        delete child;
    }
};

namespace {

template <bool NT>
__global__ __launch_bounds__(256) void hbm_probe_copy_kernel(const ldpc::vf4 *__restrict__ src, ldpc::vf4 *__restrict__ dst, size_t n4)
{
    const size_t stride = (size_t)gridDim.x * 256 * 4;
    for (size_t i = (size_t)blockIdx.x * 256 * 4 + threadIdx.x; i < n4; i += stride) {
        ldpc::vf4 v[4];
#pragma unroll
        for (int k = 0; k < 4; ++k)
            if (i + (size_t)k * 256 < n4) v[k] = NT ? __builtin_nontemporal_load(&src[i + (size_t)k * 256]) : src[i + (size_t)k * 256];
#pragma unroll
        for (int k = 0; k < 4; ++k)
            if (i + (size_t)k * 256 < n4) {
                if (NT) __builtin_nontemporal_store(v[k], &dst[i + (size_t)k * 256]);
                else dst[i + (size_t)k * 256] = v[k];
            }
    }
}

template <int V>
__global__ void summary_kernel(const int32_t *iters, const uint64_t *done, const uint64_t *fail,
                               int64_t frames, int32_t freeze, int32_t *summary)
{
    constexpr int F = 64 * V;
    const int64_t f = (int64_t)blockIdx.x * blockDim.x + threadIdx.x;
    if (f >= frames) return;
    const int64_t tile = f / F;
    const int fi = (int)(f % F);
    const int l = fi / V, v = fi % V;
    atomicMax(&summary[0], iters[f]);
    const uint64_t ok = freeze ? done[tile * V + v] : ~fail[tile * V + v];
    if ((ok >> l) & 1ull) atomicAdd(&summary[1], 1);
}

int pick_frames_per_lane(const ldpc_decoder_config &cfg, int32_t max_row_deg, int32_t max_col_deg)
{
    if (cfg.frames_per_lane) return cfg.frames_per_lane;
    int deg = cfg.algo == LDPC_ALGO_LAYERED ? max_row_deg : max_col_deg;
    if (cfg.algo == LDPC_ALGO_MS) deg = (deg + 1) / 2;
    if (cfg.max_batch >= 1024 && deg <= 8) return 4;
    if (cfg.max_batch >= 256 && deg <= ldpc::kMaxUnrolledDegree) return 2;
    return 1;
}

hipError_t span_begin(ldpc_decoder *d, hipStream_t s, int kind, int degree = 0, int64_t bytes = 0, int64_t moved = -1,
                      int lo = 0)
{
    if (!d->timing) return hipSuccess;
    if (d->spans_used == d->spans.size()) {
        TimedSpan t{};
        hipError_t e = hipEventCreate(&t.a);
        if (e != hipSuccess) return e;
        e = hipEventCreate(&t.b);
        if (e != hipSuccess) return e;
        d->spans.push_back(t);
    }
    d->spans[d->spans_used].kind = kind;
    d->spans[d->spans_used].degree = degree;
    d->spans[d->spans_used].bytes = bytes;
    d->spans[d->spans_used].moved = moved < 0 ? bytes : moved;
    d->spans[d->spans_used].lo = lo;
    return hipEventRecord(d->spans[d->spans_used].a, s);
}

hipError_t span_end(ldpc_decoder *d, hipStream_t s)
{
    if (!d->timing) return hipSuccess;
    return hipEventRecord(d->spans[d->spans_used++].b, s);
}

static inline dim3 flood_grid(const ldpc_decoder *d, unsigned blocks, unsigned tiles, int32_t *tiles_first, bool linked = false)
{
    const bool want = d->tune_tiles_first == 1 || (d->tune_tiles_first == 0 && linked);
    *tiles_first = (blocks <= 65535u && want) ? 1 : 0;
    return *tiles_first ? dim3(tiles, blocks) : dim3(blocks, tiles);
}

template <int V> int run_flooding(ldpc_decoder *d, const float *llr_dev, int64_t frames,
                                  uint8_t *out_dev, int64_t out_bytes, int32_t *iters_dev,
                                  hipStream_t s, int start_round = 1);

template <int V> int enqueue_check_phase(ldpc_decoder *d, hipStream_t s, int tiles, int64_t frames, int it, int max_iter,
                                         bool fat, const ldpc::TailRef &tr)
{
    using namespace ldpc;
    const int64_t msz = d->msg_size;
    for (auto &rc : d->row_classes) {
        if (!rc.linked) continue;
        HIP_TRY(span_begin(d, s, 4, rc.degree,
                           (2 * msz * rc.degree * rc.count + msz * 5 * rc.linked + 2 * msz * d->extra_edges) * frames,
                           msz * ((int64_t)rc.degree * rc.count + rc.linked +
                                  ((int64_t)rc.degree * rc.count - 2 * rc.linked) +
                                  (it < max_iter ? 2 * rc.linked : 0) + 2 * d->extra_edges) * frames));
        CheckArgs a{d->Q.p, d->R.p, rc.e0.p, d->done.p, d->E, rc.count, 1, rc.degree, d->ms_scale, tr};
        a.ms_offset = d->ms_offset;
        a.qpos = d->qpos.p;
        LinkArgs lk{rc.link_col.p, rc.link_pos.p, d->chan.p, d->Q.p, d->hard.p, d->N,
                    (it < max_iter) ? 1 : 0, d->tap_iter ? 1 : 0, d->extra_e0.p, d->extra_deg.p, d->n_extra, 0,
                    rc.n_big, rc.small_rows};
        a.rows_per_wave = d->link_rpw;
        const int variant = (d->tune_link_narrow == 2 && !d->link_half_fn[rc.degree]) ? 1 : d->tune_link_narrow;
        const int waves = link_chunk_count(d->link_rpw, rc.n_big, rc.small_rows, rc.count) * (variant == 1 ? V : variant == 2 ? V / 2 : 1);
        lk.link_blocks = (waves + kWavesPerBlock - 1) / kWavesPerBlock;
        const dim3 grid = flood_grid(d, lk.link_blocks + (d->n_extra + kWavesPerBlock - 1) / kWavesPerBlock, tiles, &a.tiles_first, true);
        (variant == 2 ? d->link_half_fn : variant == 1 ? (d->tune_link_deep ? d->link_deep_fn : d->link_narrow_fn) : d->link_fn)
            [rc.degree]<<<grid, kBlock, 0, s>>>(a, lk);
        HIP_TRY(span_end(d, s));
    }
    for (auto &g : d->check_groups) {
        int64_t edges = 0;
        for (int i : g.members) edges += (int64_t)d->row_classes[i].degree * d->row_classes[i].count;
        HIP_TRY(span_begin(d, s, 5, g.hi, 2 * msz * edges * frames, -1, g.lo));
        CheckArgs a{d->Q.p, d->R.p, nullptr, d->done.p, d->E, 0, (d->tune_rpw ? d->tune_rpw : 2) * (fat ? kIdleFat : 1), 0, d->ms_scale, tr};
        a.ms_offset = d->ms_offset;
        a.qpos = d->qpos.p;
        if (it == 1 && d->first_round_from_chan) { a.first_chan = d->chan.p; a.edge_col = d->edge_col.p; a.N = d->N; }
        const dim3 grid = flood_grid(d, fat ? g.blocks_fat : g.blocks, tiles, &a.tiles_first);
        d->check_group_fn[g.bucket]<<<grid, kBlock, 0, s>>>(a, fat ? g.table_fat.p : g.table.p, (int)g.members.size());
        HIP_TRY(span_end(d, s));
    }
    for (int ci : d->check_solo) {
        RowClass &rc = d->row_classes[ci];
        HIP_TRY(span_begin(d, s, 0, rc.degree, 2 * msz * rc.degree * rc.count * frames));
        CheckArgs a{d->Q.p, d->R.p, rc.e0.p, d->done.p, d->E, rc.count, 1, rc.degree, d->ms_scale, tr};
        a.ms_offset = d->ms_offset;
        a.qpos = d->qpos.p;
        if (it == 1 && d->first_round_from_chan) { a.first_chan = d->chan.p; a.edge_col = d->edge_col.p; a.N = d->N; }
        const int slotk = rc.degree <= d->max_check_unrolled ? rc.degree : 0;
        const bool narrow = slotk && (!d->tune_check_wide || rc.degree > kMaxUnrolledDegree);
        const int rpw = (d->tune_rpw ? d->tune_rpw : (narrow ? 2 : 1)) * (fat ? kIdleFat : 1);
        a.rows_per_wave = rpw;
        const int waves = ((rc.count + rpw - 1) / rpw) * (narrow ? V : 1);
        const dim3 grid = flood_grid(d, (waves + kWavesPerBlock - 1) / kWavesPerBlock, tiles, &a.tiles_first);
        (narrow ? d->check_fn : d->check_fn_wide)[slotk]<<<grid, kBlock, 0, s>>>(a);
        HIP_TRY(span_end(d, s));
    }
    return LDPC_OK;
}

template <int V> int enqueue_var_phase(ldpc_decoder *d, hipStream_t s, int tiles, int64_t frames, int it, int max_iter,
                                       bool fat, const ldpc::TailRef &tr)
{
    using namespace ldpc;
    const int64_t msz = d->msg_size;
    const int wq = (it < max_iter) ? 1 : 0;
    for (auto &g : d->var_groups) {
        int64_t units = 0;
        for (int i : g.members) units += (int64_t)((wq ? 2 : 1) * d->col_classes[i].degree + 1) * d->col_classes[i].count;
        HIP_TRY(span_begin(d, s, 6, g.hi, msz * units * frames, -1, g.lo));
        VarArgs a{d->R.p, d->Q.p, d->chan.p, d->hard.p, d->done.p, nullptr, nullptr,
                  d->E, d->N, 0, (d->tune_cpw ? d->tune_cpw : 1) * (fat ? kIdleFat : 1), wq, 0, tr};
        const dim3 grid = flood_grid(d, fat ? g.blocks_fat : g.blocks, tiles, &a.tiles_first);
        d->var_group_fn[g.bucket]<<<grid, kBlock, 0, s>>>(a, fat ? g.table_fat.p : g.table.p, (int)g.members.size());
        HIP_TRY(span_end(d, s));
    }
    for (int ci : d->var_solo) {
        ColClass &cc = d->col_classes[ci];
        HIP_TRY(span_begin(d, s, 1, cc.degree, msz * ((wq ? 2 : 1) * cc.degree + 1) * cc.count * frames));
        VarArgs a{d->R.p, d->Q.p, d->chan.p, d->hard.p, d->done.p, cc.col.p, cc.edge.p,
                  d->E, d->N, cc.count, 1, wq, cc.degree, tr};
        const int cpw = (d->tune_cpw ? d->tune_cpw : 1) * (fat ? kIdleFat : 1);
        a.cols_per_wave = cpw;
        a.q_base = cc.q_base;
        const int slotk = cc.degree <= kMaxUnrolledDegree ? cc.degree : 0;
        const int waves = (cc.count + cpw - 1) / cpw;
        const dim3 grid = flood_grid(d, (waves + kWavesPerBlock - 1) / kWavesPerBlock, tiles, &a.tiles_first);
        d->var_fn[slotk]<<<grid, kBlock, 0, s>>>(a);
        HIP_TRY(span_end(d, s));
    }
    return LDPC_OK;
}

template <int V> int compact_and_finish(ldpc_decoder *d, int64_t frames, int count, int it, hipStream_t s)
{
    using namespace ldpc;
    ldpc_decoder *c = d->child;
    while (c->child && count <= c->child->cfg.max_batch) c = c->child;
    const int cv = c->V, cf = 64 * cv;
    const unsigned ct = (unsigned)((count + cf - 1) / cf);
    const unsigned cg = ct * (unsigned)cv;
    if (cg > (unsigned)kBackWords) return fail(LDPC_ERR_STATE, "hand-over of %d frames: more than %d mask words per column", count, kBackWords);
    HIP_TRY(hipMemsetAsync(d->active.p, 0, sizeof(int32_t), s));
    compact_list_kernel<V><<<(unsigned)((frames + kBlock - 1) / kBlock), kBlock, 0, s>>>(d->done.p, frames, d->cmap.p,
                                                                                         d->active.p, d->child_capacity);
    const dim3 ge((unsigned)((d->E + kWavesPerBlock - 1) / kWavesPerBlock), cg);
    const dim3 gn((unsigned)((d->N + kWavesPerBlock - 1) / kWavesPerBlock), cg);
    const bool rowwise = count >= 128;
    const int ptiles = (int)((frames + 64 * V - 1) / (64 * V));
    if (d->msg_size == 2) {
        if (rowwise) {
            compact_gather_rows_kernel<V, _Float16><<<(unsigned)((d->E + gather_rows_per_block<_Float16>() - 1) / gather_rows_per_block<_Float16>()), kBlock, 0, s>>>((const _Float16 *)d->Q.p, (_Float16 *)c->Q.p, d->cmap.p, count, d->E, ptiles, cf, d->qpos.p, c->qpos.p);
            compact_gather_rows_kernel<V, _Float16><<<(unsigned)((d->N + gather_rows_per_block<_Float16>() - 1) / gather_rows_per_block<_Float16>()), kBlock, 0, s>>>((const _Float16 *)d->chan.p, (_Float16 *)c->chan.p, d->cmap.p, count, d->N, ptiles, cf);
        } else {
            compact_gather_kernel<V, _Float16><<<ge, kBlock, 0, s>>>((const _Float16 *)d->Q.p, (_Float16 *)c->Q.p, d->cmap.p, count, d->E, cf, d->qpos.p, c->qpos.p);
            compact_gather_kernel<V, _Float16><<<gn, kBlock, 0, s>>>((const _Float16 *)d->chan.p, (_Float16 *)c->chan.p, d->cmap.p, count, d->N, cf);
        }
    } else {
        if (rowwise) {
            compact_gather_rows_kernel<V, float><<<(unsigned)((d->E + gather_rows_per_block<float>() - 1) / gather_rows_per_block<float>()), kBlock, 0, s>>>((const float *)d->Q.p, (float *)c->Q.p, d->cmap.p, count, d->E, ptiles, cf, d->qpos.p, c->qpos.p);
            compact_gather_rows_kernel<V, float><<<(unsigned)((d->N + gather_rows_per_block<float>() - 1) / gather_rows_per_block<float>()), kBlock, 0, s>>>((const float *)d->chan.p, (float *)c->chan.p, d->cmap.p, count, d->N, ptiles, cf);
        } else {
            compact_gather_kernel<V, float><<<ge, kBlock, 0, s>>>((const float *)d->Q.p, (float *)c->Q.p, d->cmap.p, count, d->E, cf, d->qpos.p, c->qpos.p);
            compact_gather_kernel<V, float><<<gn, kBlock, 0, s>>>((const float *)d->chan.p, (float *)c->chan.p, d->cmap.p, count, d->N, cf);
        }
    }
    HIP_TRY(hipMemsetAsync(c->hard.p, 0, (size_t)ct * d->N * cv * sizeof(uint64_t), s));
    if (d->cfg.algo == LDPC_ALGO_SP) {
        if (ptiles * V <= kGatherParentWords && count <= 2 * kCompactCapacity)
            compact_hard_lds_kernel<V><<<(unsigned)((d->N + 63) / 64), kBlock, 0, s>>>(d->hard.p, c->hard.p, d->cmap.p, count, d->N, cv, ptiles, (int)cg);
        else
            compact_hard_kernel<V><<<gn, kBlock, 0, s>>>(d->hard.p, c->hard.p, d->cmap.p, count, d->N, cv);
    }
    compact_child_state_kernel<0><<<ct, 64, 0, s>>>(c->done.p, c->iters.p, count, d->cfg.max_iter, cv);
    HIP_TRY(hipGetLastError());
    c->timing = false;
    c->tap_iter = 0;
    const int rc = cv == 1 ? run_flooding<1>(c, nullptr, count, nullptr, 0, nullptr, s, it + 1)
                           : cv == 2 ? run_flooding<2>(c, nullptr, count, nullptr, 0, nullptr, s, it + 1)
                                     : run_flooding<4>(c, nullptr, count, nullptr, 0, nullptr, s, it + 1);
    if (rc) return rc;
    d->handed_to = c;
    HIP_TRY(hipMemsetAsync(d->cmoved.p, 0, d->cmoved.n * sizeof(unsigned long long), s));
    compact_inverse_kernel<V><<<(unsigned)((count + 255) / 256), 256, 0, s>>>(d->cmap.p, count, d->cinv.p, d->cmoved.p, cv);
    compact_hard_back_kernel<V><<<dim3((unsigned)((d->N + kBlock - 1) / kBlock), (unsigned)ptiles), kBlock, 0, s>>>(
        d->hard.p, c->hard.p, d->cinv.p, d->cmoved.p, d->N, cv, (int)cg);
    compact_finish_kernel<V><<<(unsigned)((count + 63) / 64), 64, 0, s>>>(d->done.p, d->iters.p, c->done.p, c->iters.p, d->cmap.p, count, cv);
    HIP_TRY(hipGetLastError());
    return LDPC_OK;
}

template <int V> int run_flooding(ldpc_decoder *d, const float *llr_dev, int64_t frames,
                                  uint8_t *out_dev, int64_t out_bytes, int32_t *iters_dev,
                                  hipStream_t s, int start_round)
{
    using namespace ldpc;
    const int F = 64 * V;
    const int tiles = (int)((frames + F - 1) / F);
    const int64_t msz = d->msg_size;
    const int max_iter = d->cfg.max_iter;
    const int rounds = d->tap_iter ? std::min(d->tap_iter, max_iter) : max_iter;
    const bool freeze = d->cfg.early_term != 0;
    const size_t slot = (size_t)d->TA * V;

    const bool resume = start_round > 1;
    HIP_TRY(hipMemsetAsync(d->failw.p, 0, d->failw.n * sizeof(uint64_t), s));
    HIP_TRY(hipMemsetAsync(d->summary.p, 0, 4 * sizeof(int32_t), s));
    d->handed_to = nullptr;
    if (!resume && d->summary_pending) {
        if (hipEventQuery(d->ev_summary) == hipSuccess) {
            d->summary_pending = false;
            d->idle_after = (d->h_summary[0] > 0 && d->h_summary[0] < max_iter) ? d->h_summary[0] + 1 : 0;
        } else {
            (void)hipGetLastError();
        }
    }
    const int idle_after = (freeze && !resume && !d->tap_iter && d->cfg.poll_interval == 0) ? d->idle_after : 0;
    const bool use_tail = d->tail_enabled && freeze && !resume && !d->tap_iter && tiles >= 4 * d->TO;
    const TailRef tr{use_tail ? d->tail_state.p : nullptr, d->T, d->TO};
    TailArgs ta{};
    if (use_tail) {
        HIP_TRY(hipMemsetAsync(d->tail_state.p, 0, 4 * sizeof(int32_t), s));
        HIP_TRY(hipMemsetAsync(d->running.p, 0, d->running.n * sizeof(int32_t), s));
        ta = TailArgs{d->tail_state.p, d->tail_map.p, d->running.p, d->done.p, d->iters.p, d->Q.p, d->chan.p, d->hard.p,
                      d->E, frames, d->N, tiles, d->T, d->TO * F, std::min(d->compact_threshold, d->TO * F), 0, max_iter};
    }

    bool q_less = d->cfg.algo == LDPC_ALGO_MS && !resume && !d->tap_iter && max_iter > 1 && d->n_extra == 0;
    for (auto &rc : d->row_classes) if (rc.linked) q_less = false;
    for (int ci : d->check_solo) if (d->row_classes[ci].degree > d->max_check_unrolled) q_less = false;
    d->first_round_from_chan = q_less;
    if (!resume) {
        HIP_TRY(span_begin(d, s, 3));
        InitArgs a{llr_dev, d->chan.p, q_less ? nullptr : d->Q.p, d->hard.p, d->col_ptr.p, d->col_qedge.p,
                   d->E, frames, d->N, d->cfg.llr_scale};
        dim3 grid((d->N + kInitCols - 1) / kInitCols, tiles);
        d->init_fn<<<grid, kBlock, 0, s>>>(a);
        StateArgs st{d->done.p, nullptr, d->iters.p, nullptr, frames, 0, max_iter, freeze ? 1 : 0};
        state_kernel<V><<<use_tail ? d->TA : tiles, 64, 0, s>>>(st);
        HIP_TRY(span_end(d, s));
    }

    int launched = start_round - 1;
    bool poll_dense = false;
    for (int it = start_round; it <= rounds; ++it) {
        const bool fat = idle_after > 0 && it > idle_after;
        {
            const int rcp = enqueue_check_phase<V>(d, s, tiles, frames, it, max_iter, fat, tr);
            if (rcp) return rcp;
        }
        {
            const int rcv = enqueue_var_phase<V>(d, s, tiles, frames, it, max_iter, fat, tr);
            if (rcv) return rcv;
        }
        launched = it;
        if (freeze || it == rounds) {
            HIP_TRY(span_begin(d, s, 3));
            uint64_t *fw = d->failw.p + (size_t)it * slot;
            const int rbk = (d->M + kBlock - 1) / kBlock;
            SyndromeArgs sa{d->row_ptr.p, d->edge_col.p, d->hard.p, fw, d->done.p, d->M, d->N,
                            d->tune_syn_xcd ? tiles : 0, rbk, tr};
            dim3 sgrid = d->tune_syn_xcd ? dim3(8 * rbk * ((tiles + 7) / 8)) : dim3(rbk, tiles);
            syndrome_kernel<V><<<sgrid, kBlock, 0, s>>>(sa);
            StateArgs st{d->done.p, fw, d->iters.p, nullptr, frames, it, max_iter, 1, tr, use_tail ? d->running.p : nullptr,
                         d->summary.p + 2};
            const bool poll = freeze && it < rounds && d->cfg.poll_interval > 0 && !d->suppress_poll &&
                              ((it % d->cfg.poll_interval) == 0 || poll_dense);
            if (poll) {
                HIP_TRY(hipMemsetAsync(d->active.p, 0, sizeof(int32_t), s));
                st.active = d->active.p;
            }
            state_kernel<V><<<tiles, 64, 0, s>>>(st);
            if (use_tail && it < rounds) {
                ta.iter = it;
                const unsigned tg = (unsigned)std::min<int64_t>(1024, d->E + 2 * (int64_t)d->N);
                if (d->msg_size == 2) tail_gather_kernel<V, _Float16><<<tg, kBlock, 0, s>>>(ta);
                else tail_gather_kernel<V, float><<<tg, kBlock, 0, s>>>(ta);
            }
            HIP_TRY(span_end(d, s));
            if (poll) {
                HIP_TRY(hipMemcpyAsync(d->h_active, d->active.p, sizeof(int32_t),
                                       hipMemcpyDeviceToHost, s));
                HIP_TRY(hipStreamSynchronize(s));
                const int running = *d->h_active;
                if (running == 0) break;
                if ((int64_t)running * 10 <= frames * 9 && d->child && tiles > 1 &&
                    (double)d->E * (double)frames * 4.0 * (double)msz > 1.5e9) poll_dense = true;
                if (d->child && running <= d->compact_threshold && (int64_t)running * 4 <= frames && tiles > 1 && !d->tap_iter) {
                    const int rc = compact_and_finish<V>(d, frames, running, it, s);
                    if (rc) return rc;
                    launched = d->handed_to->last_iterations;
                    break;
                }
            }
        }
    }
    d->last_iterations = launched;
    d->last_tiles = tiles;
    if (resume) return LDPC_OK;

    HIP_TRY(span_begin(d, s, 3));
    if (use_tail) tail_scatter_kernel<V><<<2048, kBlock, 0, s>>>(ta);
    {
        PackArgs pa{d->hard.p, out_dev, d->iters.p, iters_dev, frames, out_bytes, d->N, d->cfg.K,
                    d->cfg.pack_mode};
        if (d->cfg.pack_mode == LDPC_PACK_BYTES) {
            if (out_dev && frames) pack_kernel<V><<<pack_grid<V>(d->cfg.K, tiles), kBlock, 0, s>>>(pa);
        } else {
            const int64_t n = std::max<int64_t>(out_bytes, frames);
            dim3 grid((unsigned)((n + kBlock - 1) / kBlock));
            if (out_dev && frames) pack_kernel<V><<<grid, kBlock, 0, s>>>(pa);
        }
        summary_kernel<V><<<(unsigned)((frames + 255) / 256), 256, 0, s>>>(
            d->iters.p, d->done.p, d->failw.p, frames, 1, d->summary.p);
        if (!d->is_child && d->cfg.poll_interval == 0 && freeze && !d->summary_pending) {
            HIP_TRY(hipMemcpyAsync(d->h_summary, d->summary.p, 2 * sizeof(int32_t), hipMemcpyDeviceToHost, s));
            HIP_TRY(hipEventRecord(d->ev_summary, s));
            d->summary_pending = true;
        }
    }
    HIP_TRY(span_end(d, s));
    HIP_TRY(hipGetLastError());
    return LDPC_OK;
}

int build_classes(ldpc_decoder *d, const ldpc_graph *g)
{
    std::map<int, std::vector<int32_t>> rows_by_deg, cols_by_deg, rowids_by_deg;
    for (int32_t m = 0; m < g->M; ++m) {
        const int deg = g->row_ptr[m + 1] - g->row_ptr[m];
        if (deg > 0) { rows_by_deg[deg].push_back(g->row_ptr[m]); rowids_by_deg[deg].push_back(m); }
    }
    std::vector<char> fused_col((size_t)g->N, 0);
    d->row_classes.resize(rows_by_deg.size());
    size_t i = 0;
    for (auto &kv : rows_by_deg) {
        RowClass &rc = d->row_classes[i++];
        rc.degree = kv.first;
        rc.count = (int)kv.second.size();
        rc.h_e0 = kv.second;
        HIP_TRY(rc.e0.upload(kv.second));
        const std::vector<int32_t> &ids = rowids_by_deg[kv.first];
        const int rpw = d->link_rpw;
        if (rpw >= 2 && rc.degree >= 2 && rc.degree <= ldpc::kMaxUnrolledDegree) {
// ... 95 lines not shown
    for (int i = 0; i < (int)d->row_classes.size(); ++i) {
        RowClass &rc = d->row_classes[i];
        if (rc.linked) continue;
        if (as_extra) {
            for (int32_t e : rc.h_e0) { xe0.push_back(e); xdeg.push_back(rc.degree); d->extra_edges += rc.degree; }
            continue;
        }
        int b = -1;
        for (int k = 0; k < kCheckBuckets; ++k)
            if (rc.degree >= kCheckBucketLo[k] && rc.degree <= kCheckBucketHi[k] && rc.degree <= d->max_check_unrolled &&
                d->check_group_fn[k]) b = k;
        if (merge && b >= 0) cb[b].push_back(i); else d->check_solo.push_back(i);
    }
    if (as_extra) {
        d->n_extra = (int)xe0.size();
        HIP_TRY(d->extra_e0.upload(xe0));
        HIP_TRY(d->extra_deg.upload(xdeg));
    }
    for (int i = 0; i < (int)d->col_classes.size(); ++i) {
        const ColClass &cc = d->col_classes[i];
        int b = -1;
        for (int k = 0; k < kVarBuckets; ++k)
            if (cc.degree >= kVarBucketLo[k] && cc.degree <= kVarBucketHi[k] && d->var_group_fn[k]) b = k;
        if (merge && b >= 0) vb[b].push_back(i); else d->var_solo.push_back(i);
    }
    const int rpw = d->tune_rpw ? d->tune_rpw : 2, cpw = d->tune_cpw ? d->tune_cpw : 1;
    auto make = [&](std::vector<ClassGroup> &groups, std::vector<int> &solo, const std::vector<int> &members, int bucket,
                    int lo, int hi, bool rows) -> hipError_t {
        if (members.size() < 2) { for (int i : members) solo.push_back(i); return hipSuccess; }
        groups.emplace_back();
        ClassGroup &g = groups.back();
        g.bucket = bucket; g.lo = lo; g.hi = hi; g.members = members;
        std::vector<GroupClass> tab, tabf;
        constexpr int fatk = kIdleFat;
        for (int i : members) {
            GroupClass gc{};
            if (rows) {
                const RowClass &rc = d->row_classes[i];
                gc.degree = rc.degree; gc.count = rc.count; gc.ids = rc.e0.p; gc.edges = nullptr; gc.q_base = -1;
            } else {
                const ColClass &cc = d->col_classes[i];
                gc.degree = cc.degree; gc.count = cc.count; gc.ids = cc.col.p; gc.edges = cc.edge.p; gc.q_base = cc.q_base;
            }
            auto blocks_of = [&](int per_wave) {
                const int waves = ((gc.count + per_wave - 1) / per_wave) * (rows ? V / d->check_group_width : 1);
                return (waves + ldpc::kWavesPerBlock - 1) / ldpc::kWavesPerBlock;
            };
            gc.block_begin = g.blocks;
            tab.push_back(gc);
            g.blocks += blocks_of(rows ? rpw : cpw);
            gc.block_begin = g.blocks_fat;
            tabf.push_back(gc);
            g.blocks_fat += blocks_of((rows ? rpw : cpw) * fatk);
        }
        const hipError_t e = g.table.upload(tab);
        return e != hipSuccess ? e : g.table_fat.upload(tabf);
    };
    for (int k = 0; k < kCheckBuckets; ++k) HIP_TRY(make(d->check_groups, d->check_solo, cb[k], k, kCheckBucketLo[k], kCheckBucketHi[k], true));
    for (int k = 0; k < kVarBuckets; ++k) HIP_TRY(make(d->var_groups, d->var_solo, vb[k], k, kVarBucketLo[k], kVarBucketHi[k], false));
    return LDPC_OK;
}

int setup_flooding(ldpc_decoder *d, const ldpc_graph *g, size_t TF)
{
    const ldpc_decoder_config *cfg = &d->cfg;
    d->msg_size = cfg->msg_dtype == LDPC_MSG_F16 ? 2 : 4;
    HIP_TRY(d->chan.alloc(TF * d->N * d->msg_size));
    HIP_TRY(d->Q.alloc(TF * (size_t)d->E * d->msg_size));
    HIP_TRY(d->R.alloc(TF * (size_t)d->E * d->msg_size));
    int rc = build_classes(d, g);
    if (rc) return rc;
    ldpc::FloodFns fns;
    if (cfg->algo == LDPC_ALGO_SP) ldpc::fill_flood_sp(d->V, &fns);
    else if (d->ms_corr && cfg->msg_dtype == LDPC_MSG_F16) ldpc::fill_flood_msc16(d->V, &fns);
    else if (d->ms_corr) ldpc::fill_flood_msc(d->V, &fns);
    else if (cfg->msg_dtype == LDPC_MSG_F16) ldpc::fill_flood_ms16(d->V, &fns);
    else ldpc::fill_flood_ms(d->V, &fns);
    memcpy(d->check_fn, fns.check, sizeof fns.check);
    memcpy(d->check_fn_wide, fns.check_wide, sizeof fns.check_wide);
    memcpy(d->link_fn, fns.link, sizeof fns.link);
    memcpy(d->link_narrow_fn, fns.link_narrow, sizeof fns.link_narrow);
    memcpy(d->link_deep_fn, fns.link_deep, sizeof fns.link_deep);
    memcpy(d->link_half_fn, fns.link_half, sizeof fns.link_half);
    memcpy(d->var_fn, fns.var, sizeof fns.var);
    memcpy(d->check_group_fn, fns.check_group, sizeof fns.check_group);
    d->check_group_width = fns.check_group_width;
    memcpy(d->var_group_fn, fns.var_group, sizeof fns.var_group);
    d->init_fn = fns.init;
    d->max_check_unrolled = fns.max_check_unrolled;
    return plan_launches(d);
}

template <int V> int calibrate_link(ldpc_decoder *d)
{
    using namespace ldpc;
    RowClass *rcp = nullptr;
    for (auto &rc : d->row_classes) if (rc.linked) rcp = &rc;
    if (!rcp || !d->link_fn[rcp->degree] || !d->link_narrow_fn[rcp->degree]) return LDPC_OK;
    RowClass &rc = *rcp;
    const int tiles = d->T;
    hipStream_t s = d->stream;
    HIP_TRY(hipMemsetAsync(d->Q.p, 0, d->Q.n, s));
    HIP_TRY(hipMemsetAsync(d->chan.p, 0, d->chan.n, s));
    HIP_TRY(hipMemsetAsync(d->done.p, 0, d->done.n * sizeof(uint64_t), s));
    hipEvent_t ev[2] = {nullptr, nullptr};
    HIP_TRY(hipEventCreate(&ev[0]));
    HIP_TRY(hipEventCreate(&ev[1]));
    float best[3] = {1e30f, 1e30f, 1e30f};
    const int candidates = d->link_half_fn[rc.degree] ? 3 : 2;
    hipError_t err = hipSuccess;
    for (int rep = 0; rep < 4 && err == hipSuccess; ++rep) {
        for (int nar = 0; nar < candidates && err == hipSuccess; ++nar) {
            CheckArgs a{d->Q.p, d->R.p, rc.e0.p, d->done.p, d->E, rc.count, d->link_rpw, rc.degree, d->ms_scale,
                        TailRef{nullptr, 0, 0}};
            a.ms_offset = d->ms_offset;
            a.qpos = d->qpos.p;
            LinkArgs lk{rc.link_col.p, rc.link_pos.p, d->chan.p, d->Q.p, d->hard.p, d->N, 1, 0, nullptr, nullptr, 0, 0,
                        rc.n_big, rc.small_rows};
            const int waves = link_chunk_count(d->link_rpw, rc.n_big, rc.small_rows, rc.count) * (nar == 1 ? V : nar == 2 ? V / 2 : 1);
            lk.link_blocks = (waves + kWavesPerBlock - 1) / kWavesPerBlock;
            const dim3 grid = flood_grid(d, lk.link_blocks, tiles, &a.tiles_first, true);
            err = hipEventRecord(ev[0], s);
            (nar == 2 ? d->link_half_fn : nar == 1 ? d->link_narrow_fn : d->link_fn)[rc.degree]<<<grid, kBlock, 0, s>>>(a, lk);
            if (err == hipSuccess) err = hipEventRecord(ev[1], s);
            if (err == hipSuccess) err = hipEventSynchronize(ev[1]);
            float ms = 0;
            if (err == hipSuccess) err = hipEventElapsedTime(&ms, ev[0], ev[1]);
            if (err == hipSuccess && rep > 0 && ms < best[nar]) best[nar] = ms;
        }
    }
    (void)hipEventDestroy(ev[0]);
    (void)hipEventDestroy(ev[1]);
    if (err != hipSuccess) return fail(LDPC_ERR_HIP, "link calibration: %s", hipGetErrorString(err));
    HIP_TRY(hipGetLastError());
    int pick = 0;
    for (int k = 0; k < candidates; ++k) { d->link_cal_ms[k] = best[k]; if (best[k] < best[pick]) pick = k; }
    d->tune_link_narrow = pick;
    d->link_calibrated = true;
    return LDPC_OK;
}

template <int V> int time_check_phase(ldpc_decoder *d, float *ms_out)
{
    hipStream_t s = d->stream;
    HIP_TRY(hipMemsetAsync(d->Q.p, 0, d->Q.n, s));
    HIP_TRY(hipMemsetAsync(d->chan.p, 0, d->chan.n, s));
    HIP_TRY(hipMemsetAsync(d->done.p, 0, d->done.n * sizeof(uint64_t), s));
    hipEvent_t ev[2] = {nullptr, nullptr};
    HIP_TRY(hipEventCreate(&ev[0]));
    HIP_TRY(hipEventCreate(&ev[1]));
    float best = 1e30f;
    hipError_t err = hipSuccess;
    int rc = LDPC_OK;
    for (int rep = 0; rep < 4 && err == hipSuccess && rc == LDPC_OK; ++rep) {
        err = hipEventRecord(ev[0], s);
        rc = enqueue_check_phase<V>(d, s, d->T, (int64_t)d->T * d->F, 1, d->cfg.max_iter, false, ldpc::TailRef{nullptr, 0, 0});
        if (rc == LDPC_OK)
            rc = enqueue_var_phase<V>(d, s, d->T, (int64_t)d->T * d->F, 1, d->cfg.max_iter, false, ldpc::TailRef{nullptr, 0, 0});
        if (err == hipSuccess) err = hipEventRecord(ev[1], s);
        if (err == hipSuccess) err = hipEventSynchronize(ev[1]);
        float ms = 0;
        if (err == hipSuccess) err = hipEventElapsedTime(&ms, ev[0], ev[1]);
        if (err == hipSuccess && rep > 0 && ms < best) best = ms;
    }
    (void)hipEventDestroy(ev[0]);
    (void)hipEventDestroy(ev[1]);
// ... 411 lines not shown
    return LDPC_OK;
}

int ldpc_decoder_create_multi(const ldpc_graph *g, const ldpc_decoder_config *cfg, const int32_t *devices,
                              int32_t n_devices, ldpc_decoder **out)
{
    if (!out) return fail(LDPC_ERR_ARG, "out is NULL");
    *out = nullptr;
    if (!g || !cfg) return fail(LDPC_ERR_ARG, "graph/config is NULL");
    if (!devices || n_devices <= 0 || n_devices > 64) return fail(LDPC_ERR_ARG, "devices[] must hold 1..64 ordinals");
    ldpc_decoder_config cfg_full;
    if (int rc = config_in(cfg, &cfg_full)) return rc;
    cfg = &cfg_full;
    ldpc_decoder *grp = new (std::nothrow) ldpc_decoder;
    if (!grp) return fail(LDPC_ERR_NOMEM, "out of memory");
    std::unique_ptr<ldpc_decoder> guard(grp);
    for (int32_t i = 0; i < n_devices; ++i) {
        ldpc_decoder_config c = *cfg;
        c.device = devices[i];
        ldpc_decoder *sh = nullptr;
        const int rc = ldpc_decoder_create(g, &c, &sh);
        if (rc) return rc;
        grp->shards.push_back(sh);
        grp->shard_workers.emplace_back(new (std::nothrow) ldpc::Worker([] { return g_err; }));
        if (!grp->shard_workers.back() || !grp->shard_workers.back()->start())
            return fail(LDPC_ERR_NOMEM, "cannot start the host thread of device-list entry %d", i);
    }
    grp->cfg = *cfg;
    grp->cfg.device = devices[0];
    grp->M = g->M; grp->N = g->N; grp->E = g->E;
    *out = guard.release();
    return LDPC_OK;
}

int ldpc_decode_device(ldpc_decoder *d, const float *llr_dev, int64_t frames, uint8_t *out_dev,
                       int64_t out_bytes, int32_t *iters_dev, void *stream)
{
    if (!d) return fail(LDPC_ERR_ARG, "decoder is NULL");
    if (!d->shards.empty())
        return fail(LDPC_ERR_STATE, "a multi-device handle decodes host buffers only (ldpc_decode): device "
                    "pointers belong to one device");
    if (frames < 0 || frames > d->cfg.max_batch)
        return fail(LDPC_ERR_ARG, "frames=%lld outside [0, max_batch=%d]", (long long)frames,
                    d->cfg.max_batch);
    if (frames == 0) { d->last_frames = 0; d->have_last = false; return LDPC_OK; }
    if (!llr_dev) return fail(LDPC_ERR_ARG, "llr is NULL");
    const int64_t need = ldpc_out_bytes(d->cfg.K, frames, d->cfg.pack_mode);
    if (out_dev && out_bytes < need && d->cfg.pack_mode == LDPC_PACK_BITS)
        return fail(LDPC_ERR_ARG, "out_bytes=%lld < %lld", (long long)out_bytes, (long long)need);
    HIP_TRY(hipSetDevice(d->cfg.device));
    hipStream_t s = (hipStream_t)stream;
    d->timing = d->timing_every > 0 && (d->timing_calls++ % d->timing_every) == 0;
    d->last_stream = s;
    d->last_frames = frames;
    d->call.valid = false;
    HIP_TRY(hipEventRecord(d->ev_begin, s));
    if (out_dev) HIP_TRY(hipMemsetAsync(out_dev, 0, (size_t)std::min(out_bytes, need), s));
    int rc;
    if (d->use_fused) {
        ldpc::FusedRun run{llr_dev, frames, out_dev, std::min(out_bytes, need), iters_dev, d->cfg.K,
                           d->cfg.max_iter, d->tap_iter, d->cfg.early_term, d->summary.p,
                           d->cfg.algo == LDPC_ALGO_MS_FUSED ? 1 : (d->cfg.algo == LDPC_ALGO_MS ? 2 : (d->cfg.algo == LDPC_ALGO_SP ? 3 : 0)),
                           d->cfg.llr_scale, ldpc::tune_pick(d->tune.fused_loop, false) ? 1 : 0,
                           ldpc::tune_pick(d->tune.fused_pack, true) ? 0 : 1};
        hipError_t e = span_begin(d, s, 2, 0, (int64_t)frames * (4 * d->N + d->cfg.K / 8));
        if (e == hipSuccess)
            e = d->use_ldsp ? ldpc::engine_ldsp_run(&d->ldsp, run, s, &d->last_iterations)
                            : ldpc::engine_fused_run(&d->fused, run, s, &d->last_iterations);
        if (e == hipSuccess) e = span_end(d, s);
        rc = (e == hipSuccess) ? LDPC_OK : fail(LDPC_ERR_HIP, "fused decode: %s", hipGetErrorString(e));
    } else if (d->cfg.algo == LDPC_ALGO_LAYERED || d->cfg.algo == LDPC_ALGO_LAYERED_HOST) {
        ldpc::LayeredRun run;
        run.span_begin = [](void *c, hipStream_t st, int kind, int deg, int64_t bytes) {
            return span_begin((ldpc_decoder *)c, st, kind, deg, bytes);
        };
        run.span_end = [](void *c, hipStream_t st) { return span_end((ldpc_decoder *)c, st); };
        run.span_ctx = d;
        run.llr_dev = llr_dev; run.frames = frames; run.out_dev = out_dev;
        run.out_bytes = std::min(out_bytes, need); run.iters_dev = iters_dev;
        run.K = d->cfg.K; run.max_iter = d->cfg.max_iter; run.tap_iter = d->tap_iter;
        run.early_term = d->cfg.early_term; run.pack_mode = d->cfg.pack_mode;
        run.hard = d->hard.p; run.failw = d->failw.p; run.done = d->done.p; run.iters = d->iters.p;
        run.row_ptr = d->row_ptr.p; run.edge_col = d->edge_col.p; run.summary = d->summary.p;
        hipError_t e = ldpc::engine_layered_run(&d->layered, run, s, &d->last_iterations);
        rc = (e == hipSuccess) ? LDPC_OK
                               : fail(LDPC_ERR_HIP, "layered decode: %s", hipGetErrorString(e));
    } else if (d->V == 1) rc = run_flooding<1>(d, llr_dev, frames, out_dev, std::min(out_bytes, need), iters_dev, s);
    else if (d->V == 2) rc = run_flooding<2>(d, llr_dev, frames, out_dev, std::min(out_bytes, need), iters_dev, s);
    else rc = run_flooding<4>(d, llr_dev, frames, out_dev, std::min(out_bytes, need), iters_dev, s);
    if (rc) return rc;
    HIP_TRY(hipEventRecord(d->ev_end, s));
    d->have_last = true;
    return LDPC_OK;
}

namespace {

constexpr size_t kStageBytes = (size_t)4 << 20;
constexpr size_t kRingChunk = (size_t)8 << 20;
constexpr int kRingChunks = 4;

enum InputMode { kInputDirect = 0, kInputStaged = 1, kInputLock = 2 };

InputMode resolve_input_mode(const ldpc_decoder_config &cfg, const void *p, size_t bytes)
{
    if (ldpc::PageLockRegistry::instance().caller_locked(p, (const uint8_t *)p + bytes - 1)) return kInputDirect;
    return cfg.host_input == LDPC_HOST_INPUT_LOCK_PAGES ? kInputLock : kInputStaged;
}

int ensure_stager(ldpc_decoder *d)
{
    if (d->stager) return LDPC_OK;
    if (d->ring.empty()) d->ring.resize(kRingChunks);
    for (auto &c : d->ring) {
        if (!c.h) HIP_TRY(hipHostMalloc((void **)&c.h, kRingChunk, hipHostMallocDefault));
        if (!c.ev) HIP_TRY(hipEventCreateWithFlags(&c.ev, hipEventDisableTiming));
    }
    const int threads = d->cfg.host_copy_threads > 0 ? d->cfg.host_copy_threads : 4;
    while ((int)d->copy_helpers.size() < threads - 1) {
        std::unique_ptr<ldpc::Worker> w(new (std::nothrow) ldpc::Worker([] { return g_err; }));
        if (!w || !w->start()) return fail(LDPC_ERR_NOMEM, "cannot start a copy thread");
        d->copy_helpers.push_back(std::move(w));
    }
    d->copy_jobs.resize(d->copy_helpers.size());
    std::unique_ptr<ldpc::Worker> st(new (std::nothrow) ldpc::Worker([] { return g_err; }));
    if (!st || !st->start()) return fail(LDPC_ERR_NOMEM, "cannot start the staging thread");
    d->stager = std::move(st);
    return LDPC_OK;
}

void ring_fill(ldpc_decoder *d, uint8_t *dst, const uint8_t *src, size_t n)
{
    const size_t parts = d->copy_helpers.size() + 1;
    if (parts == 1 || n < ((size_t)1 << 20)) { memcpy(dst, src, n); return; }
    const size_t per = ((n + parts - 1) / parts + 4095) & ~(size_t)4095;
    size_t used = 0;
    for (size_t i = 0; i < d->copy_helpers.size(); ++i) {
        const size_t lo = (i + 1) * per;
        if (lo >= n) break;
        const size_t len = std::min(per, n - lo);
        d->copy_jobs[i].fn = [dst, src, lo, len]() -> int { memcpy(dst + lo, src + lo, len); return 0; };
        d->copy_helpers[i]->submit(&d->copy_jobs[i]);
        ++used;
    }
    memcpy(dst, src, std::min(per, n));
    for (size_t i = 0; i < used; ++i) (void)d->copy_helpers[i]->wait(&d->copy_jobs[i]);
}

hipError_t staged_copy(ldpc_decoder *d, uint8_t *dst, const uint8_t *src, size_t bytes)
{
    for (size_t o = 0; o < bytes; o += kRingChunk) {
        const size_t n = std::min(kRingChunk, bytes - o);
        auto &c = d->ring[d->ring_next++ % d->ring.size()];
        hipError_t e = c.used ? hipEventSynchronize(c.ev) : hipSuccess;
        if (e != hipSuccess) return e;
        ring_fill(d, c.h, src + o, n);
        e = hipMemcpyAsync(dst + o, c.h, n, hipMemcpyHostToDevice, d->copy_stream);
        if (e == hipSuccess) e = hipEventRecord(c.ev, d->copy_stream);
        if (e != hipSuccess) return e;
        c.used = true;
    }
    return hipSuccess;
}

int decode_host(ldpc_decoder *d, const float *llr_host, int64_t frames, uint8_t *out_host,
                int64_t out_bytes, int32_t *iters, InputMode mode)
// ... 322 lines not shown
    st->frame_rounds = 0;
    if (!d->use_fused && d->cfg.algo != LDPC_ALGO_LAYERED && d->cfg.algo != LDPC_ALGO_LAYERED_HOST) {
        st->frame_rounds = d->cfg.early_term ? (int64_t)summary[2] * d->F
                                             : (int64_t)d->last_iterations * d->last_tiles * d->F;
        for (const ldpc_decoder *p = d->handed_to; p; p = p->handed_to) {
            int32_t cs[4] = {0, 0, 0, 0};
            HIP_TRY(hipMemcpy(cs, p->summary.p, sizeof cs, hipMemcpyDeviceToHost));
            st->frame_rounds += (int64_t)cs[2] * p->F;
        }
    }
    if (d->call.valid) {
        st->iterations_launched = d->call.iterations;
        st->batch_time = d->call.batch_time;
        st->frames = d->call.frames;
        st->frames_converged = d->call.converged;
        st->frame_rounds = d->call.frame_rounds;
    }
    for (size_t i = 0; i < d->spans_used; ++i) {
        float ms = 0;
        HIP_TRY(hipEventElapsedTime(&ms, d->spans[i].a, d->spans[i].b));
        const int kind = d->spans[i].kind;
        if (kind == 0 || kind == 4 || kind == 5) { st->ms_check += ms; ++st->launches_check; }
        else if (kind == 1 || kind == 2 || kind == 6) { st->ms_var += ms; ++st->launches_var; }
        else st->ms_other += ms;
    }
    return LDPC_OK;
}

int ldpc_decoder_kernel_times(ldpc_decoder *d, ldpc_kernel_time *out, int32_t capacity, int32_t *count)
{
    if (!d || !out || !count || capacity <= 0) return fail(LDPC_ERR_ARG, "bad arguments");
    *count = 0;
    if (!d->shards.empty()) return ldpc_decoder_kernel_times(d->shards[0], out, capacity, count);
    if (!d->have_last) return fail(LDPC_ERR_STATE, "no decode call to report on");
    HIP_TRY(hipSetDevice(d->cfg.device));
    HIP_TRY(hipEventSynchronize(d->ev_end));
    const char *phase_name[] = {"check_kernel", "var_kernel", d->ms_corr ? "layer_corr_kernel" : "layer_kernel", "other",
                                d->tune_link_narrow == 2 ? "check_link_half_kernel"
                                : d->tune_link_narrow ? "check_link_narrow_kernel" : "check_link_kernel"};
    static const char *algo_name_f32[] = {"sp", "ms", "layered", "ms_fused", "layered_host"};
    static const char *algo_name_f16[] = {"sp16", "ms16", "layered16", "ms_fused16", "layered_host16"};
    static const char *algo_name_corr_f32[] = {"sp", "msc", "layered", "ms_fused", "layered_host"};
    static const char *algo_name_corr_f16[] = {"sp16", "msc16", "layered16", "ms_fused16", "layered_host16"};
    const char **algo_name = d->ms_corr ? (d->msg_size == 2 ? algo_name_corr_f16 : algo_name_corr_f32)
                                        : (d->msg_size == 2 ? algo_name_f16 : algo_name_f32);
    for (size_t i = 0; i < d->spans_used; ++i) {
        const TimedSpan &sp = d->spans[i];
        float ms = 0;
        HIP_TRY(hipEventElapsedTime(&ms, sp.a, sp.b));
        const int phase = (sp.kind == 4 || sp.kind == 5) ? 0 : (sp.kind == 6 ? 1 : sp.kind);
        char name[64];
        if (sp.kind == 3) snprintf(name, sizeof name, "other");
        else if (d->use_fused && d->use_ldsp)
            snprintf(name, sizeof name, "%s[%dx%d,%d]", d->cfg.algo == LDPC_ALGO_LAYERED
                     ? (d->ms_corr ? "layered_ldsp_corr_kernel" : "layered_ldsp_kernel")
                     : (d->ms_corr ? "flood_ldsp_corr_kernel" : "flood_ldsp_kernel"),
                     d->ldsp.grid, d->ldsp.block, d->ldsp.wg_frames);
        else if (d->use_fused)
            snprintf(name, sizeof name, "%s", d->cfg.algo == LDPC_ALGO_SP ? "fused_sp_kernel"
                     : d->cfg.algo == LDPC_ALGO_LAYERED ? "fused_layered_kernel" : "fused_flood_kernel");
        else if (sp.kind == 5 || sp.kind == 6)
            snprintf(name, sizeof name, "%s<%s,%d-%d,%d>", sp.kind == 5 ? "check_group_kernel" : "var_group_kernel",
                     algo_name[d->cfg.algo], sp.lo, sp.degree, d->V);
        else snprintf(name, sizeof name, "%s<%s,%d,%d>", phase_name[sp.kind], algo_name[d->cfg.algo], sp.degree, d->V);
        int k = 0;
        for (; k < *count; ++k)
            if (!strcmp(out[k].name, name)) break;
        if (k == *count) {
            if (*count == capacity) continue;
            ++*count;
            memset(&out[k], 0, sizeof out[k]);
            out[k].phase = phase;
            out[k].degree = sp.degree;
            memcpy(out[k].name, name, sizeof name);
        }
        ++out[k].launches;
        out[k].ms_total += ms;
        out[k].bytes_total += sp.bytes;
        out[k].bytes_moved += sp.moved;
    }
    return LDPC_OK;
}

int ldpc_decoder_link_form(ldpc_decoder *d, int32_t *form, int32_t *calibrated, float ms[3])
{
    if (!d) return fail(LDPC_ERR_ARG, "decoder is NULL");
    if (!d->shards.empty()) return ldpc_decoder_link_form(d->shards[0], form, calibrated, ms);
    bool linked = false;
    for (auto &rc : d->row_classes) linked = linked || rc.linked;
    if (form) *form = linked ? d->tune_link_narrow : -1;
    if (calibrated) *calibrated = d->link_calibrated ? 1 : 0;
    if (ms) for (int k = 0; k < 3; ++k) ms[k] = d->link_calibrated && d->link_cal_ms[k] < 1e29f ? d->link_cal_ms[k] : 0.0f;
    return LDPC_OK;
}

int ldpc_decoder_placement(ldpc_decoder *d, int32_t *candidates, int32_t *kept, float ms[16])
{
    if (!d) return fail(LDPC_ERR_ARG, "decoder is NULL");
    if (!d->shards.empty()) return ldpc_decoder_placement(d->shards[0], candidates, kept, ms);
    if (candidates) *candidates = d->place_candidates;
    if (kept) *kept = d->place_kept;
    if (ms) for (int k = 0; k < 16; ++k) ms[k] = k < d->place_candidates ? d->place_ms[k] : 0.0f;
    return LDPC_OK;
}

int ldpc_decoder_array_addresses(ldpc_decoder *d, uint64_t out[4])
{
    if (!d || !out) return fail(LDPC_ERR_ARG, "decoder/out is NULL");
    if (!d->shards.empty()) return ldpc_decoder_array_addresses(d->shards[0], out);
    out[0] = (uint64_t)(uintptr_t)d->Q.p; out[1] = (uint64_t)(uintptr_t)d->R.p;
    out[2] = (uint64_t)(uintptr_t)d->chan.p; out[3] = (uint64_t)(uintptr_t)d->hard.p;
    return LDPC_OK;
}

int ldpc_decoder_set_tap(ldpc_decoder *d, int32_t iter)
{
    if (!d) return fail(LDPC_ERR_ARG, "decoder is NULL");
    if (iter < 0) return fail(LDPC_ERR_ARG, "iter < 0");
    if (!d->shards.empty()) return fail(LDPC_ERR_STATE, "debug taps need a single-device handle");
    d->tap_iter = iter;
    return LDPC_OK;
}

int ldpc_decoder_dump(ldpc_decoder *d, int32_t which, float *host_out, int64_t count)
{
    if (!d || !host_out) return fail(LDPC_ERR_ARG, "decoder/host_out is NULL");
    if (!d->shards.empty()) return fail(LDPC_ERR_STATE, "debug taps need a single-device handle");
    if (!d->have_last) return fail(LDPC_ERR_STATE, "no decode call to dump");
    HIP_TRY(hipSetDevice(d->cfg.device));
    wait_for_own_work(d);
    const int64_t frames = d->last_frames;
    const int V = d->V, F = d->F;
    const int tiles = (int)((frames + F - 1) / F);
    if (d->use_fused && d->cfg.algo == LDPC_ALGO_SP) {
        if (!d->fused.dump_p) return fail(LDPC_ERR_STATE, "fused dump needs set_tap() before the decode");
        const int64_t per = (which == 0 || which == 1) ? d->E : d->N;
        if (which < 0 || which > 3 || count != frames * per) return fail(LDPC_ERR_ARG, "bad `which`/count");
        if (which == 3) {
            std::vector<uint8_t> b((size_t)count);
            HIP_TRY(hipMemcpy(b.data(), d->fused.dump_b, (size_t)count, hipMemcpyDeviceToHost));
            for (int64_t i = 0; i < count; ++i) host_out[i] = (float)b[i];
            return LDPC_OK;
        }
        const float *src = which == 0 ? d->fused.dump_r : (which == 1 ? d->fused.dump_q : d->fused.dump_p);
        HIP_TRY(hipMemcpy(host_out, src, (size_t)count * sizeof(float), hipMemcpyDeviceToHost));
        return LDPC_OK;
    }
    if (d->use_fused) {
        const float *dump_r = d->use_ldsp ? d->ldsp.dump_r : d->fused.dump_r;
        const float *dump_p = d->use_ldsp ? d->ldsp.dump_p : d->fused.dump_p;
        const float *src = which == 0 ? dump_r : (which == 2 ? dump_p : nullptr);
        const int64_t per = which == 0 ? d->E : d->N;
        if (which == 3) {
            if (!dump_p || count != frames * d->N) return fail(LDPC_ERR_ARG, "fused dump needs set_tap() and count = frames*N");
            HIP_TRY(hipMemcpy(host_out, dump_p, (size_t)count * sizeof(float), hipMemcpyDeviceToHost));
            const bool notpos = d->cfg.algo == LDPC_ALGO_MS;
            for (int64_t i = 0; i < count; ++i)
                host_out[i] = (notpos ? !(host_out[i] > 0.0f) : (host_out[i] < 0.0f)) ? 1.0f : 0.0f;
            return LDPC_OK;
        }
        if (!src || count != frames * per) return fail(LDPC_ERR_ARG, "fused dump: set_tap() first; which in {0,2,3}");
        HIP_TRY(hipMemcpy(host_out, src, (size_t)count * sizeof(float), hipMemcpyDeviceToHost));
        return LDPC_OK;
    }
    if (d->cfg.algo == LDPC_ALGO_LAYERED || d->cfg.algo == LDPC_ALGO_LAYERED_HOST) {
        hipError_t e = ldpc::layered_dump(&d->layered, which, host_out, count, frames, d->hard.p,
// ... 191 lines not shown
```

### myldpccppapi_amd/csrc/tune.hpp

```cpp
#pragma once

#include "../../include/ldpc_hip.h"

namespace ldpc {

struct Tune {
    int fused = 0, ldsp = 0, ldsp_ext = 0, ldsp_pack = 0, link_narrow = 0, check_wide = 0, syn_xcd = 0,
        fused_pack = 0, fused_loop = 0, device_tail = 0, merge = 0, link_deep = 0, link_half = 0, link_guided = 0, tiles_first = 0;
    int rows_per_wave = 0, cols_per_wave = 0;
    int link_rows = 0;
    int compact = 0;
    int ldsp_grid = 0, ldsp_per_cu = 0, ldsp_waves = 0;
    int place = 0;
    int q_order = 0;
};

inline Tune tune_from_config(const ldpc_decoder_config &c)
{
    Tune t;
    auto f = [&](int field) { return (c.tune_flags >> field) & 3; };
    t.fused = f(LDPC_TUNE_FUSED);
    t.ldsp = f(LDPC_TUNE_LDSP);
    t.ldsp_ext = f(LDPC_TUNE_LDSP_EXT);
    t.ldsp_pack = f(LDPC_TUNE_LDSP_PACK);
    t.link_narrow = f(LDPC_TUNE_LINK_NARROW);
    t.check_wide = f(LDPC_TUNE_CHECK_WIDE);
    t.syn_xcd = f(LDPC_TUNE_SYN_XCD);
    t.fused_pack = f(LDPC_TUNE_FUSED_PACK);
    t.fused_loop = f(LDPC_TUNE_FUSED_LOOP);
    t.device_tail = f(LDPC_TUNE_DEVICE_TAIL);
    t.merge = f(LDPC_TUNE_MERGE);
    t.link_deep = f(LDPC_TUNE_LINK_DEEP);
    t.link_half = f(LDPC_TUNE_LINK_HALF);
    t.link_guided = f(LDPC_TUNE_LINK_GUIDED);
    t.tiles_first = f(LDPC_TUNE_TILES_FIRST);
    t.rows_per_wave = c.tune_rows_per_wave;
    t.cols_per_wave = c.tune_cols_per_wave;
    t.link_rows = c.tune_link_rows;
    t.compact = c.tune_compact;
    t.ldsp_grid = c.tune_ldsp_grid;
    t.ldsp_per_cu = c.tune_ldsp_shape & 255;
    t.ldsp_waves = (c.tune_ldsp_shape >> 8) & 255;
    t.place = c.tune_place;
    t.q_order = c.tune_q_order;
    return t;
}

inline bool tune_pick(int tri, bool dflt) { return tri == 1 ? true : (tri == 2 ? false : dflt); }
inline bool tune_forced_on(int tri) { return tri == 1; }
inline bool tune_forced_off(int tri) { return tri == 2; }

inline bool tune_valid(const ldpc_decoder_config &c)
{
    for (int field = 0; field <= LDPC_TUNE_TILES_FIRST; field += 2)
        if (((c.tune_flags >> field) & 3) == 3) return false;
    if (c.tune_flags >> (LDPC_TUNE_TILES_FIRST + 2)) return false;
    return c.tune_rows_per_wave >= 0 && c.tune_rows_per_wave <= 4096 && c.tune_cols_per_wave >= 0 &&
           c.tune_cols_per_wave <= 4096 && c.tune_link_rows >= -1 && c.tune_link_rows <= 4096 &&
           c.tune_compact >= -1 && c.tune_ldsp_grid >= 0 && c.tune_ldsp_shape >= 0 && c.tune_ldsp_shape < 65536 &&
           c.tune_place >= 0 && c.tune_place <= 8 && c.host_input >= 0 && c.host_input <= 2 && c.host_copy_threads >= 0 && c.host_copy_threads <= 16 &&
           c.tune_q_order >= -1 && c.tune_q_order <= 1;
}

}
```

Baseline: 1084 Mbit/s.

## Feed first SP check round from channel values and batch syndrome gathers

Extends the first-round-from-channel shortcut to sum-product decoding. In the first iteration the check kernels, including a new FIRST variant of the link kernel, read channel probabilities per column and convert them to the initial q on the fly. This avoids reading a materialised Q array, and the init pass that writes it may be skipped. Separately, the syndrome kernel now gathers edge columns and hard bits in chunks of eight to expose more memory-level parallelism, with masking at the row end. Both are on by default and can be switched off through a new side-tuning word; the change also adds more kernel variants and recomputation in round one.

```diff
diff --git a/include/ldpc_hip.h b/include/ldpc_hip.h
--- a/include/ldpc_hip.h
+++ b/include/ldpc_hip.h
@@ -67,6 +67,11 @@
     float ms_scale;
     float ms_offset;
 } ldpc_decoder_config;
+
+enum ldpc_side_field {
+    LDPC_SIDE_SYN_BATCH = 0,
+    LDPC_SIDE_FIRST_CHAN = 2
+};
 
 enum ldpc_tune_field {
     LDPC_TUNE_FUSED = 0,
@@ -144,6 +149,10 @@
 
 int ldpc_decoder_link_form(ldpc_decoder *d, int32_t *form, int32_t *calibrated, float ms[3]);
 
+int ldpc_decoder_first_round_from_chan(ldpc_decoder *d, int32_t *taken, int32_t *child);
+
+int ldpc_decoder_set_side_tuning(ldpc_decoder *d, int32_t side);
+
 int ldpc_decoder_placement(ldpc_decoder *d, int32_t *candidates, int32_t *kept, float ms[16]);
 int ldpc_decoder_array_addresses(ldpc_decoder *d, uint64_t out[4]);
 
diff --git a/myldpccppapi_amd/_lib.py b/myldpccppapi_amd/_lib.py
--- a/myldpccppapi_amd/_lib.py
+++ b/myldpccppapi_amd/_lib.py
@@ -51,7 +51,7 @@
     "ldpc_decoder_create_multi", "ldpc_shard_range", "ldpc_decoder_destroy", "ldpc_decode", "ldpc_decode_device", "ldpc_out_bytes",
     "ldpc_decoder_set_timing", "ldpc_decoder_stats", "ldpc_decoder_kernel_times", "ldpc_decoder_set_tap",
     "ldpc_decoder_dump", "ldpc_awgn_device", "ldpc_count_errors_device", "ldpc_hbm_probe_device", "ldpc_hbm_sustained_device",
-    "ldpc_host_block_plan", "ldpc_host_locked_ranges", "ldpc_decoder_link_form", "ldpc_decoder_placement", "ldpc_decoder_array_addresses",
+    "ldpc_host_block_plan", "ldpc_host_locked_ranges", "ldpc_decoder_link_form", "ldpc_decoder_first_round_from_chan", "ldpc_decoder_set_side_tuning", "ldpc_decoder_placement", "ldpc_decoder_array_addresses",
     "ldpc_parity_structure", "ldpc_encoder_create", "ldpc_encoder_destroy", "ldpc_encode_device", "ldpc_encode", "ldpc_code_bytes",
 )
 
@@ -107,6 +107,8 @@
     L.ldpc_decoder_array_addresses.argtypes = [vp, ctypes.POINTER(ctypes.c_uint64)]
     L.ldpc_decoder_placement.argtypes = [vp, i32p, i32p, ctypes.POINTER(ctypes.c_float)]
     L.ldpc_decoder_link_form.argtypes = [vp, i32p, i32p, ctypes.POINTER(ctypes.c_float)]
+    L.ldpc_decoder_first_round_from_chan.argtypes = [vp, i32p, i32p]
+    L.ldpc_decoder_set_side_tuning.argtypes = [vp, ctypes.c_int32]
     L.ldpc_parity_structure.argtypes = [vp, ctypes.c_int32, ctypes.c_int32, i32p]
     L.ldpc_encoder_create.argtypes = [vp, ctypes.c_int32, ctypes.c_int32, ctypes.c_int32, ctypes.c_int32, ctypes.POINTER(vp)]
     L.ldpc_encoder_destroy.argtypes = [vp]
diff --git a/myldpccppapi_amd/capi.py b/myldpccppapi_amd/capi.py
--- a/myldpccppapi_amd/capi.py
+++ b/myldpccppapi_amd/capi.py
@@ -18,6 +18,7 @@
 TUNE_FIELDS = {"fused": 0, "ldsp": 2, "ldsp_ext": 4, "ldsp_pack": 6, "link_narrow": 8, "check_wide": 10,
                "syn_xcd": 12, "fused_pack": 14, "fused_loop": 16, "device_tail": 18, "merge": 20, "link_deep": 22, "link_half": 24,
                "link_guided": 26, "tiles_first": 28}
+SIDE_FIELDS = {"syn_batch": 0, "first_chan": 2}
 TUNE_INTS = ("rows_per_wave", "cols_per_wave", "link_rows", "compact", "ldsp_grid", "ldsp_per_cu", "ldsp_waves", "place", "q_order")
 
 
@@ -27,6 +28,8 @@
         if k in TUNE_FIELDS:
             if v is not None:
                 flags |= (1 if v else 2) << TUNE_FIELDS[k]
+        elif k in SIDE_FIELDS:
+            pass
         elif k == "ldsp_per_cu":
             shape |= int(v) & 255
         elif k == "ldsp_waves":
@@ -36,6 +39,14 @@
         else:
             raise KeyError("unknown tuning field %r" % k)
     cfg.tune_flags, cfg.tune_ldsp_shape = flags, shape
+
+
+def side_word(tune):
+    side = 0
+    for k, v in (tune or {}).items():
+        if k in SIDE_FIELDS and v is not None:
+            side |= (1 if v else 2) << SIDE_FIELDS[k]
+    return side
 
 
 def hbm_probe(device=0, nbytes=1 << 30, reps=5, by_policy=False):
@@ -176,6 +187,8 @@
             devs = (ctypes.c_int32 * len(devices))(*[int(x) for x in devices])
             _lib.check(L.ldpc_decoder_create_multi(graph._h, ctypes.byref(cfg), devs, len(devices),
                                                    ctypes.byref(self._h)))
+        if side_word(tune):
+            self.set_side_tuning(side_word(tune))
 
     def decode(self, llr, want_iters=True):
         L = _lib.load()
@@ -216,6 +229,14 @@
             return None
         return {"form": ("wide", "narrow", "half")[form.value], "chosen_by_measurement": bool(cal.value),
                 "ms_per_launch": {"wide": round(ms[0], 4), "narrow": round(ms[1], 4), "half": round(ms[2], 4)}}
+
+    def set_side_tuning(self, side):
+        _lib.check(_lib.load().ldpc_decoder_set_side_tuning(self._h, int(side)))
+
+    def first_round_from_chan(self):
+        taken, child = ctypes.c_int32(0), ctypes.c_int32(-1)
+        _lib.check(_lib.load().ldpc_decoder_first_round_from_chan(self._h, ctypes.byref(taken), ctypes.byref(child)))
+        return bool(taken.value), (None if child.value < 0 else bool(child.value))
 
     def placement(self):
         n, kept = ctypes.c_int32(0), ctypes.c_int32(0)
diff --git a/myldpccppapi_amd/csrc/flood_kernels.hpp b/myldpccppapi_amd/csrc/flood_kernels.hpp
--- a/myldpccppapi_amd/csrc/flood_kernels.hpp
+++ b/myldpccppapi_amd/csrc/flood_kernels.hpp
@@ -164,6 +164,20 @@
     return tiles_first ? GridPos{(int)blockIdx.x, (int)blockIdx.y} : GridPos{(int)blockIdx.y, (int)blockIdx.x};
 }
 
+template <int ALGO> __device__ __forceinline__ float first_q(float c)
+{
+    return ALGO == kAlgoSP ? c / (1.0f + c) - 1.0f / (1.0f + c) : c;
+}
+template <int ALGO, int D, int W> __device__ __forceinline__ void first_q_row(float (&x)[D][W])
+{
+    if (ALGO != kAlgoSP) return;
+#pragma unroll
+    for (int k = 0; k < D; ++k) {
+#pragma unroll
+        for (int w = 0; w < W; ++w) x[k][w] = first_q<ALGO>(x[k][w]);
+    }
+}
+
 template <int D, int V>
 __device__ __forceinline__ void check_sp(const float (&x)[D][V], float (&out)[D][V])
 {
@@ -241,14 +255,14 @@
     const T *Qu = static_cast<const T *>(a.Q) + (size_t)tile * (size_t)a.E * F;
     T *Rt = static_cast<T *>(a.R) + (size_t)tile * (size_t)a.E * F + lane_off;
 
-    const T *Ct = (ALGO != kAlgoSP && a.first_chan)
-                      ? static_cast<const T *>(a.first_chan) + (size_t)tile * (size_t)a.N * F + lane_off : nullptr;
+    const T *Ct = a.first_chan ? static_cast<const T *>(a.first_chan) + (size_t)tile * (size_t)a.N * F + lane_off : nullptr;
     for (int r = r_begin; r < r_end; ++r) {
         const int e0 = a.cls_e0[r];
         float x[D][W], out[D][W];
-        if (ALGO != kAlgoSP && Ct) {
+        if (Ct) {
 #pragma unroll
             for (int k = 0; k < D; ++k) vload<W>(x[k], Ct + (size_t)a.edge_col[e0 + k] * F);
+            first_q_row<ALGO, D, W>(x);
         } else {
             int sl[D];
             row_slots<D>(a.qpos, e0, lane, sl);
@@ -263,9 +277,19 @@
 
 template <int ALGO, int V, typename T>
 __device__ __forceinline__ void check_row_generic(const T *Qu, unsigned lane_off, T *Rt, int e0, int D,
-                                                  const int32_t *__restrict__ qpos, const MsCorr &c)
+                                                  const int32_t *__restrict__ qpos, const MsCorr &c,
+                                                  const T *Cu = nullptr, const int32_t *__restrict__ edge_col = nullptr)
 {
     constexpr size_t F = 64 * V;
+    auto load_q = [&](float (&xj)[V], int e) {
+        if (Cu) {
+            vload<V>(xj, Cu + (size_t)__builtin_amdgcn_readfirstlane(edge_col[e]) * F + lane_off);
+#pragma unroll
+            for (int v = 0; v < V; ++v) xj[v] = first_q<ALGO>(xj[v]);
+        } else {
+            vload<V>(xj, Qu + (size_t)edge_slot(qpos, e) * F + lane_off);
+        }
+    };
     if (ALGO != kAlgoSP) {
         float m1[V], m2[V];
         int idx[V];
@@ -274,7 +298,7 @@
         for (int v = 0; v < V; ++v) { m1[v] = 1000.0f; m2[v] = 1000.0f; idx[v] = -1; par[v] = 0; }
         for (int j = 0; j < D; ++j) {
             float xj[V];
-            vload<V>(xj, Qu + (size_t)edge_slot(qpos, e0 + j) * F + lane_off);
+            load_q(xj, e0 + j);
 #pragma unroll
             for (int v = 0; v < V; ++v) {
                 const float m = __builtin_fabsf(xj[v]);
@@ -289,7 +313,7 @@
         }
         for (int k = 0; k < D; ++k) {
             float xk[V], o[V];
-            vload<V>(xk, Qu + (size_t)edge_slot(qpos, e0 + k) * F + lane_off);
+            load_q(xk, e0 + k);
 #pragma unroll
             for (int v = 0; v < V; ++v) {
                 const float b = (k == idx[v]) ? m2[v] : m1[v];
@@ -308,7 +332,7 @@
         for (int j = 0; j < D; ++j) {
             if (j == k) continue;
             float xj[V];
-            vload<V>(xj, Qu + (size_t)edge_slot(qpos, e0 + j) * F + lane_off);
+            load_q(xj, e0 + j);
 #pragma unroll
             for (int v = 0; v < V; ++v) p[v] *= xj[v];
         }
@@ -331,7 +355,9 @@
     const int r_end = min(r_begin + a.rows_per_wave, a.n_rows);
     const T *Qu = static_cast<const T *>(a.Q) + (size_t)tile * (size_t)a.E * F;
     T *Rt = static_cast<T *>(a.R) + (size_t)tile * (size_t)a.E * F + (size_t)lane * V;
-    for (int r = r_begin; r < r_end; ++r) check_row_generic<ALGO, V, T>(Qu, (unsigned)lane * V, Rt, a.cls_e0[r], a.degree, a.qpos, ms_corr_of(a));
+    const T *Cu = a.first_chan ? static_cast<const T *>(a.first_chan) + (size_t)tile * (size_t)a.N * F : nullptr;
+    for (int r = r_begin; r < r_end; ++r)
+        check_row_generic<ALGO, V, T>(Qu, (unsigned)lane * V, Rt, a.cls_e0[r], a.degree, a.qpos, ms_corr_of(a), Cu, a.edge_col);
 }
 
 struct GroupClass {
@@ -354,9 +380,10 @@
     for (int r = r_begin; r < r_end; ++r) {
         const int e0 = e0s[r];
         float x[D][W], out[D][W];
-        if (ALGO != kAlgoSP && Ct) {
+        if (Ct) {
 #pragma unroll
             for (int k = 0; k < D; ++k) vload<W>(x[k], Ct + (size_t)edge_col[e0 + k] * F);
+            first_q_row<ALGO, D, W>(x);
         } else {
             int sl[D];
             row_slots<D>(qpos, e0, lane, sl);
@@ -403,8 +430,7 @@
     const unsigned lane_off = (unsigned)sub * 64 * W + (unsigned)lane * W;
     const T *Qu = static_cast<const T *>(a.Q) + (size_t)tile * (size_t)a.E * F;
     T *Rt = static_cast<T *>(a.R) + (size_t)tile * (size_t)a.E * F + lane_off;
-    const T *Ct = (ALGO != kAlgoSP && a.first_chan)
-                      ? static_cast<const T *>(a.first_chan) + (size_t)tile * (size_t)a.N * F + lane_off : nullptr;
+    const T *Ct = a.first_chan ? static_cast<const T *>(a.first_chan) + (size_t)tile * (size_t)a.N * F + lane_off : nullptr;
     CheckDispatch<ALGO, V, T, DHI, DLO, W>::run(cls[c].degree, Qu, lane_off, Rt, cls[c].ids, r_begin, r_end, Ct, a.edge_col, a.qpos, ms_corr_of(a));
 }
 
@@ -418,7 +444,10 @@
     int32_t tiles;
     int32_t row_blocks;
     TailRef tail;
+    int32_t serial = 0;
 };
+
+constexpr int kSynChunk = 8;
 
 template <int V> __global__ __launch_bounds__(kBlock) void syndrome_kernel(const SyndromeArgs a)
 {
@@ -440,10 +469,31 @@
 #pragma unroll
     for (int v = 0; v < V; ++v) s[v] = 0;
     if (m < a.M) {
-        for (int p = a.row_ptr[m]; p < a.row_ptr[m + 1]; ++p) {
-            const int c = a.edge_col[p];
-#pragma unroll
-            for (int v = 0; v < V; ++v) s[v] ^= hard_t[(size_t)c * V + v];
+        const int p0 = a.row_ptr[m], p1 = a.row_ptr[m + 1];
+        if (a.serial) {
+            for (int p = p0; p < p1; ++p) {
+                const int c = a.edge_col[p];
+#pragma unroll
+                for (int v = 0; v < V; ++v) s[v] ^= hard_t[(size_t)c * V + v];
+            }
+        } else {
+            for (int p = p0; p < p1; p += kSynChunk) {
+                int c[kSynChunk];
+#pragma unroll
+                for (int k = 0; k < kSynChunk; ++k) c[k] = a.edge_col[min(p + k, p1 - 1)];
+                uint64_t w[kSynChunk][V];
+#pragma unroll
+                for (int k = 0; k < kSynChunk; ++k) {
+#pragma unroll
+                    for (int v = 0; v < V; ++v) w[k][v] = hard_t[(size_t)c[k] * V + v];
+                }
+#pragma unroll
+                for (int k = 0; k < kSynChunk; ++k) {
+                    const uint64_t keep = (p + k < p1) ? ~0ull : 0ull;
+#pragma unroll
+                    for (int v = 0; v < V; ++v) s[v] ^= w[k][v] & keep;
+                }
+            }
         }
     }
     __shared__ uint64_t part[kWavesPerBlock][V];
@@ -552,7 +602,7 @@
     return n_big + (rest > 0 ? (rest + small_rows - 1) / small_rows : 0);
 }
 
-template <int ALGO, int V, typename T>
+template <int ALGO, int V, typename T, bool FIRST = false>
 __device__ __forceinline__ void link_extra_rows(const CheckArgs &a, const LinkArgs &g, int tile, int block)
 {
     constexpr size_t F = 64 * V;
@@ -561,7 +611,8 @@
     if (w >= g.n_extra) return;
     const T *Qu = static_cast<const T *>(a.Q) + (size_t)tile * (size_t)a.E * F;
     T *Rt = static_cast<T *>(a.R) + (size_t)tile * (size_t)a.E * F + (size_t)lane * V;
-    check_row_generic<ALGO, V, T>(Qu, (unsigned)lane * V, Rt, g.extra_e0[w], g.extra_deg[w], a.qpos, ms_corr_of(a));
+    const T *Cu = FIRST ? static_cast<const T *>(a.first_chan) + (size_t)tile * (size_t)a.N * F : nullptr;
+    check_row_generic<ALGO, V, T>(Qu, (unsigned)lane * V, Rt, g.extra_e0[w], g.extra_deg[w], a.qpos, ms_corr_of(a), Cu, a.edge_col);
 }
 
 #ifdef LDPC_LINK_WIDE_WAVES
@@ -569,7 +620,7 @@
 #else
 #define LDPC_LINK_WIDE_ATTR
 #endif
-template <int ALGO, int D, int V, typename T>
+template <int ALGO, int D, int V, typename T, bool FIRST = false>
 __global__ __launch_bounds__(kBlock) LDPC_LINK_WIDE_ATTR void check_link_kernel(const CheckArgs a, const LinkArgs g)
 {
     constexpr size_t F = 64 * V;
@@ -577,7 +628,7 @@
     const GridPos gp = grid_pos(a.tiles_first);
     const int tile = tile_select<V>(a.tail, a.done, gp.row);
     if (tile < 0) return;
-    if (gp.block >= g.link_blocks) { link_extra_rows<ALGO, V, T>(a, g, tile, gp.block); return; }
+    if (gp.block >= g.link_blocks) { link_extra_rows<ALGO, V, T, FIRST>(a, g, tile, gp.block); return; }
     const int wave = gp.block * kWavesPerBlock + wave_id_in_block();
     int r_begin, r_end;
     link_chunk_rows(wave, a.rows_per_wave, g.n_big, g.small_rows, a.n_rows, &r_begin, &r_end);
@@ -601,13 +652,24 @@
     int qc[D], qn[D];
 #pragma unroll
     for (int k = 0; k < D; ++k) qc[k] = qn[k] = 0;
+    auto request_chan = [&](int e0) {
+        int col[D];
+        row_slots<D>(a.edge_col, e0, lane, col);
+#pragma unroll
+        for (int k = 0; k < D; ++k) vload<V>(x[k], chan_t + (size_t)col[k] * F);
+    };
     if (r_begin < r_end) {
         row_slots<D>(a.qpos, a.cls_e0[r_begin], lane, qc);
-#pragma unroll
-        for (int k = 0; k < D; ++k) vload<V>(x[k], Qt + (size_t)qc[k] * F + lane_q);
+        if (FIRST) {
+            request_chan(a.cls_e0[r_begin]);
+        } else {
+#pragma unroll
+            for (int k = 0; k < D; ++k) vload<V>(x[k], Qt + (size_t)qc[k] * F + lane_q);
+        }
     }
     for (int r = r_begin; r < r_end; ++r) {
         const int e0 = a.cls_e0[r];
+        if (FIRST) first_q_row<ALGO, D, V>(x);
         const int next_col = (r + 1 < r_end) ? g.link_col[r] : -1;
         const int pos = g.link_pos[r];
         const int ka = next_col >= 0 ? (pos & 255) : -1;
@@ -623,8 +685,12 @@
         float out[D][V];
         if (ALGO == kAlgoSP) check_sp<D, V>(x, out); else if (ALGO == kAlgoMS) check_ms<D, V>(x, out); else check_ms<D, V, true, T>(x, out, ms_corr_of(a));
         if (r + 1 < r_end) {
-#pragma unroll
-            for (int k = 0; k < D; ++k) vload<V>(x[k], Qt + (size_t)qn[k] * F + lane_q);
+            if (FIRST) {
+                request_chan(a.cls_e0[r + 1]);
+            } else {
+#pragma unroll
+                for (int k = 0; k < D; ++k) vload<V>(x[k], Qt + (size_t)qn[k] * F + lane_q);
+            }
         }
 #pragma unroll
         for (int k = 0; k < D; ++k)
@@ -1257,7 +1323,7 @@
             if (ALGO == kAlgoSP) {
                 const float t = ldpc_expf(a.llr_scale * y);
                 ch[v] = t;
-                q[v] = t / (1.0f + t) - 1.0f / (1.0f + t);
+                q[v] = first_q<kAlgoSP>(t);
             } else {
                 ch[v] = y;
                 q[v] = y;
diff --git a/myldpccppapi_amd/csrc/flood_tables.hpp b/myldpccppapi_amd/csrc/flood_tables.hpp
--- a/myldpccppapi_amd/csrc/flood_tables.hpp
+++ b/myldpccppapi_amd/csrc/flood_tables.hpp
@@ -22,6 +22,7 @@
     LinkFn link_narrow[kMaxUnrolledDegree + 1] = {};
     LinkFn link_deep[kMaxUnrolledDegree + 1] = {};
     LinkFn link_half[kMaxUnrolledDegree + 1] = {};
+    LinkFn link_first[kMaxUnrolledDegree + 1] = {};
     VarFn var[kMaxUnrolledDegree + 1] = {};
     CheckGroupFn check_group[kCheckBuckets] = {};
     int check_group_width = 1;
diff --git a/myldpccppapi_amd/csrc/flood_tables_impl.hpp b/myldpccppapi_amd/csrc/flood_tables_impl.hpp
--- a/myldpccppapi_amd/csrc/flood_tables_impl.hpp
+++ b/myldpccppapi_amd/csrc/flood_tables_impl.hpp
@@ -39,25 +39,32 @@
 template <int ALGO, typename T, int D> struct LinkHalf<ALGO, 4, T, D> {
     static LinkFn get() { return check_link_narrow_kernel<ALGO, D, 4, T, 2>; }
 };
+template <int ALGO, int V, typename T, int D> struct LinkFirst {
+    static LinkFn get() { return nullptr; }
+};
+template <int V, typename T, int D> struct LinkFirst<kAlgoSP, V, T, D> {
+    static LinkFn get() { return check_link_kernel<kAlgoSP, D, V, T, true>; }
+};
 template <int ALGO, int V, typename T, int D> struct LinkTable {
-    static void fill(LinkFn *t, LinkFn *tn, LinkFn *td, LinkFn *th)
+    static void fill(LinkFn *t, LinkFn *tn, LinkFn *td, LinkFn *th, LinkFn *tf)
     {
         t[D] = check_link_kernel<ALGO, D, V, T>;
         tn[D] = check_link_narrow_kernel<ALGO, D, V, T>;
         td[D] = check_link_narrow2_kernel<ALGO, D, V, T>;
         th[D] = LinkHalf<ALGO, V, T, D>::get();
-        LinkTable<ALGO, V, T, D - 1>::fill(t, tn, td, th);
+        tf[D] = LinkFirst<ALGO, V, T, D>::get();
+        LinkTable<ALGO, V, T, D - 1>::fill(t, tn, td, th, tf);
     }
 };
 template <int ALGO, int V, typename T> struct LinkTable<ALGO, V, T, 1> {
-    static void fill(LinkFn *, LinkFn *, LinkFn *, LinkFn *) {}
+    static void fill(LinkFn *, LinkFn *, LinkFn *, LinkFn *, LinkFn *) {}
 };
 
 template <int ALGO, int V, typename T> void fill_v(FloodFns *f)
 {
     constexpr int DM = kMaxUnrolledDegree;
     FloodTable<ALGO, V, T, DM>::fill(f->check, f->check_wide, f->var);
-    LinkTable<ALGO, V, T, DM>::fill(f->link, f->link_narrow, f->link_deep, f->link_half);
+    LinkTable<ALGO, V, T, DM>::fill(f->link, f->link_narrow, f->link_deep, f->link_half, f->link_first);
     constexpr int GW = (sizeof(T) == 2 && V == 4) ? 2 : 1;
     f->check_group_width = GW;
     f->check_group[0] = check_group_kernel<ALGO, V, T, 1, 8, GW>;
diff --git a/myldpccppapi_amd/csrc/layered_kernels.hpp b/myldpccppapi_amd/csrc/layered_kernels.hpp
--- a/myldpccppapi_amd/csrc/layered_kernels.hpp
+++ b/myldpccppapi_amd/csrc/layered_kernels.hpp
@@ -200,6 +200,7 @@
     int32_t *iters;
     const int32_t *row_ptr, *edge_col;
     int32_t *summary;
+    int32_t syn_serial = 0;
 };
 
 #ifdef LDPC_ENGINE_LAYERED
@@ -276,7 +277,7 @@
         }
         if (!r.early_term && it != rounds) continue;
         uint64_t *fw = r.failw + (size_t)it * slot;
-        SyndromeArgs sa{r.row_ptr, r.edge_col, r.hard, fw, r.done, pl->M, pl->N, 0, 0};
+        SyndromeArgs sa{r.row_ptr, r.edge_col, r.hard, fw, r.done, pl->M, pl->N, 0, 0, TailRef{nullptr, 0, 0}, r.syn_serial};
         dim3 sgrid((pl->M + kBlock - 1) / kBlock, tiles);
         syndrome_kernel<V><<<sgrid, kBlock, 0, s>>>(sa);
         StateArgs st{r.done, fw, r.iters, nullptr, r.frames, it, r.max_iter, 1};
diff --git a/myldpccppapi_amd/csrc/ldpc_hip.hip b/myldpccppapi_amd/csrc/ldpc_hip.hip
--- a/myldpccppapi_amd/csrc/ldpc_hip.hip
+++ b/myldpccppapi_amd/csrc/ldpc_hip.hip
@@ -186,6 +186,7 @@
     LinkFn link_narrow_fn[ldpc::kMaxUnrolledDegree + 1] = {};
     LinkFn link_deep_fn[ldpc::kMaxUnrolledDegree + 1] = {};
     LinkFn link_half_fn[ldpc::kMaxUnrolledDegree + 1] = {};
+    LinkFn link_first_fn[ldpc::kMaxUnrolledDegree + 1] = {};
     int tune_link_deep = 0;
     ldpc::Tune tune;
     int tune_link_narrow = 1;
@@ -260,11 +261,13 @@
     int tune_rpw = 0, tune_cpw = 0;
     int tune_syn_xcd = 1;
     int tune_check_wide = 0;
+    int tune_syn_batch = 1;
     int32_t last_iterations = 0;
     int64_t last_frames = 0;
     DevBuf<int32_t> summary;
     ldpc_decoder *handed_to = nullptr;
     bool first_round_from_chan = false;
+    int tune_first_chan = 1;
     int32_t last_tiles = 0;
 
     std::vector<ldpc_decoder *> shards;
@@ -401,11 +404,13 @@
                     (it < max_iter) ? 1 : 0, d->tap_iter ? 1 : 0, d->extra_e0.p, d->extra_deg.p, d->n_extra, 0,
                     rc.n_big, rc.small_rows};
         a.rows_per_wave = d->link_rpw;
-        const int variant = (d->tune_link_narrow == 2 && !d->link_half_fn[rc.degree]) ? 1 : d->tune_link_narrow;
+        const bool first = it == 1 && d->first_round_from_chan;
+        if (first) { a.first_chan = d->chan.p; a.edge_col = d->edge_col.p; a.N = d->N; }
+        const int variant = first ? 0 : (d->tune_link_narrow == 2 && !d->link_half_fn[rc.degree]) ? 1 : d->tune_link_narrow;
         const int waves = link_chunk_count(d->link_rpw, rc.n_big, rc.small_rows, rc.count) * (variant == 1 ? V : variant == 2 ? V / 2 : 1);
         lk.link_blocks = (waves + kWavesPerBlock - 1) / kWavesPerBlock;
         const dim3 grid = flood_grid(d, lk.link_blocks + (d->n_extra + kWavesPerBlock - 1) / kWavesPerBlock, tiles, &a.tiles_first, true);
-        (variant == 2 ? d->link_half_fn : variant == 1 ? (d->tune_link_deep ? d->link_deep_fn : d->link_narrow_fn) : d->link_fn)
+        (first ? d->link_first_fn : variant == 2 ? d->link_half_fn : variant == 1 ? (d->tune_link_deep ? d->link_deep_fn : d->link_narrow_fn) : d->link_fn)
             [rc.degree]<<<grid, kBlock, 0, s>>>(a, lk);
         HIP_TRY(span_end(d, s));
     }
@@ -567,9 +572,16 @@
                       d->E, frames, d->N, tiles, d->T, d->TO * F, std::min(d->compact_threshold, d->TO * F), 0, max_iter};
     }
 
-    bool q_less = d->cfg.algo == LDPC_ALGO_MS && !resume && !d->tap_iter && max_iter > 1 && d->n_extra == 0;
-    for (auto &rc : d->row_classes) if (rc.linked) q_less = false;
-    for (int ci : d->check_solo) if (d->row_classes[ci].degree > d->max_check_unrolled) q_less = false;
+    bool q_less = d->tune_first_chan && !resume && !d->tap_iter && max_iter > 1;
+    if (d->cfg.algo == LDPC_ALGO_SP) {
+        for (auto &rc : d->row_classes) if (rc.linked && !d->link_first_fn[rc.degree]) q_less = false;
+    } else if (d->cfg.algo == LDPC_ALGO_MS) {
+        if (d->n_extra) q_less = false;
+        for (auto &rc : d->row_classes) if (rc.linked) q_less = false;
+        for (int ci : d->check_solo) if (d->row_classes[ci].degree > d->max_check_unrolled) q_less = false;
+    } else {
+        q_less = false;
+    }
     d->first_round_from_chan = q_less;
     if (!resume) {
         HIP_TRY(span_begin(d, s, 3));
@@ -600,7 +612,7 @@
             uint64_t *fw = d->failw.p + (size_t)it * slot;
             const int rbk = (d->M + kBlock - 1) / kBlock;
             SyndromeArgs sa{d->row_ptr.p, d->edge_col.p, d->hard.p, fw, d->done.p, d->M, d->N,
-                            d->tune_syn_xcd ? tiles : 0, rbk, tr};
+                            d->tune_syn_xcd ? tiles : 0, rbk, tr, d->tune_syn_batch ? 0 : 1};
             dim3 sgrid = d->tune_syn_xcd ? dim3(8 * rbk * ((tiles + 7) / 8)) : dim3(rbk, tiles);
             syndrome_kernel<V><<<sgrid, kBlock, 0, s>>>(sa);
             StateArgs st{d->done.p, fw, d->iters.p, nullptr, frames, it, max_iter, 1, tr, use_tail ? d->running.p : nullptr,
@@ -862,6 +874,7 @@
     memcpy(d->link_narrow_fn, fns.link_narrow, sizeof fns.link_narrow);
     memcpy(d->link_deep_fn, fns.link_deep, sizeof fns.link_deep);
     memcpy(d->link_half_fn, fns.link_half, sizeof fns.link_half);
+    memcpy(d->link_first_fn, fns.link_first, sizeof fns.link_first);
     memcpy(d->var_fn, fns.var, sizeof fns.var);
     memcpy(d->check_group_fn, fns.check_group, sizeof fns.check_group);
     d->check_group_width = fns.check_group_width;
@@ -1439,6 +1452,7 @@
         run.early_term = d->cfg.early_term; run.pack_mode = d->cfg.pack_mode;
         run.hard = d->hard.p; run.failw = d->failw.p; run.done = d->done.p; run.iters = d->iters.p;
         run.row_ptr = d->row_ptr.p; run.edge_col = d->edge_col.p; run.summary = d->summary.p;
+        run.syn_serial = d->tune_syn_batch ? 0 : 1;
         hipError_t e = ldpc::engine_layered_run(&d->layered, run, s, &d->last_iterations);
         rc = (e == hipSuccess) ? LDPC_OK
                                : fail(LDPC_ERR_HIP, "layered decode: %s", hipGetErrorString(e));
@@ -1927,6 +1941,28 @@
     return LDPC_OK;
 }
 
+int ldpc_decoder_first_round_from_chan(ldpc_decoder *d, int32_t *taken, int32_t *child)
+{
+    if (!d) return fail(LDPC_ERR_ARG, "decoder is NULL");
+    if (!d->shards.empty()) return ldpc_decoder_first_round_from_chan(d->shards[0], taken, child);
+    if (taken) *taken = d->first_round_from_chan ? 1 : 0;
+    if (child) *child = d->handed_to ? (d->handed_to->first_round_from_chan ? 1 : 0) : -1;
+    return LDPC_OK;
+}
+
+int ldpc_decoder_set_side_tuning(ldpc_decoder *d, int32_t side)
+{
+    if (!d) return fail(LDPC_ERR_ARG, "decoder is NULL");
+    if (!ldpc::side_valid(side)) return fail(LDPC_ERR_ARG, "side tuning word 0x%x out of range", (unsigned)side);
+    for (ldpc_decoder *sh : d->shards)
+        if (int rc = ldpc_decoder_set_side_tuning(sh, side)) return rc;
+    for (ldpc_decoder *p = d; p; p = p->child) {
+        p->tune_syn_batch = ldpc::tune_pick((side >> LDPC_SIDE_SYN_BATCH) & 3, true);
+        p->tune_first_chan = ldpc::tune_pick((side >> LDPC_SIDE_FIRST_CHAN) & 3, true);
+    }
+    return LDPC_OK;
+}
+
 int ldpc_decoder_link_form(ldpc_decoder *d, int32_t *form, int32_t *calibrated, float ms[3])
 {
     if (!d) return fail(LDPC_ERR_ARG, "decoder is NULL");
diff --git a/myldpccppapi_amd/csrc/tune.hpp b/myldpccppapi_amd/csrc/tune.hpp
--- a/myldpccppapi_amd/csrc/tune.hpp
+++ b/myldpccppapi_amd/csrc/tune.hpp
@@ -46,6 +46,13 @@
     return t;
 }
 
+inline bool side_valid(int32_t side)
+{
+    for (int field = 0; field <= LDPC_SIDE_FIRST_CHAN; field += 2)
+        if (((side >> field) & 3) == 3) return false;
+    return (side >> (LDPC_SIDE_FIRST_CHAN + 2)) == 0;
+}
+
 inline bool tune_pick(int tri, bool dflt) { return tri == 1 ? true : (tri == 2 ? false : dflt); }
 inline bool tune_forced_on(int tri) { return tri == 1; }
 inline bool tune_forced_off(int tri) { return tri == 2; }
```

After: 1079 Mbit/s. No clear change (-0.4%).
